# YanhaoWu/UMGen

Hardware: AMD Instinct MI355X
Metric: scene_tokens_per_sec (higher is better)
Workload: dtype bf16; 1 GPU; UMGen_large --infer_task video, 5-frame rollout, 1 scene(s)/GPU, T=20 history frames, top-k 5/5/16 sampling, rule_constrain; scenes_per_gpu=1, history_frames=20, input_history_frames=20

## Files before the change

umgen_amd/_lib.py:

```python
from __future__ import annotations

import ctypes as C
import os
import shutil
import subprocess

HERE = os.path.dirname(os.path.abspath(__file__))
CSRC = os.path.join(HERE, "csrc")
LIB_PATH = os.environ.get("UMGEN_LIB_PATH") or os.path.join(HERE, "libumgen_hip.so")
SOURCES = ["engine.hip", "gemm.hip", "gemm256.hip", "attn.hip", "gemv.hip", "oar_engine.hip", "oar_engine_wide.hip", "decode_batched.hip", "rowops.hip", "frame.hip", "tokenizers.hip", "vqdec.hip", "debug_api.hip"]
EXPORTS = ["umgen_create", "umgen_load_tensor", "umgen_finalize_weights", "umgen_rollout", "umgen_frame",
           "umgen_set_profiling", "umgen_get_timings", "umgen_last_error", "umgen_version", "umgen_destroy",
           "umgen_tokenize_ego", "umgen_detokenize_ego", "umgen_tokenize_boxes", "umgen_detokenize_boxes",
           "umgen_vq_create", "umgen_vq_load_tensor", "umgen_vq_finalize", "umgen_vq_decode", "umgen_vq_last_error", "umgen_vq_destroy",
           "umgen_dbg_linear", "umgen_dbg_attn_spatial", "umgen_dbg_attn_temporal", "umgen_dbg_attn_decode", "umgen_dbg_gemv", "umgen_dbg_gemm_bench", "umgen_dbg_oar_step", "umgen_dbg_sample_topk", "umgen_dbg_batched_layer_bench",
           "umgen_dbg_rows", "umgen_dbg_attn_decode_batched", "umgen_dbg_sample", "umgen_dbg_collision",
           "umgen_dbg_gemv_modes", "umgen_dbg_gemv_resid", "umgen_dbg_attn_partial", "umgen_dbg_decode_layer"]

HEADERS = ("common.h", "kernels.h", "frame.h", "oar_common.h", "bg_queue.h", "bg_worker.h", "gemm256_body.h", "attn_body.h", "rowops_body.h", "frame_body.h")

PREC_FP32, PREC_BF16, PREC_FP16 = 0, 1, 2
DT_F32, DT_BF16, DT_F16, DT_F64 = 0, 1, 2, 3


class Config(C.Structure):
    _fields_ = [(n, C.c_int32) for n in (
        "abi_version", "n_embd", "n_head", "n_ego_tar_layer", "n_ego_ca_layer", "n_map_tar_layer", "n_box_tar_layer",
        "n_tar_layer", "n_oar_layer", "pose_vocab", "map_vocab", "bbox3d_vocab", "img_vocab", "aux_vocab",
        "n_map_embd", "n_img_embd", "max_frame_len", "task_num", "task_id", "precision", "max_batch",
        "max_cond_frames", "device", "use_graphs")]


class VQConfig(C.Structure):
    _fields_ = [("n_embed", C.c_int32), ("embed_dim", C.c_int32), ("z_channels", C.c_int32), ("ch", C.c_int32), ("out_ch", C.c_int32),
                ("n_levels", C.c_int32), ("ch_mult", C.c_int32 * 8), ("num_res_blocks", C.c_int32), ("n_attn_res", C.c_int32),
                ("attn_resolutions", C.c_int32 * 4), ("resolution", C.c_int32), ("post_quant_ks", C.c_int32), ("post_quant_pad", C.c_int32),
                ("token_h", C.c_int32), ("token_w", C.c_int32), ("device", C.c_int32)]


class Sampling(C.Structure):
    _fields_ = [("method", C.c_int32), ("top_k", C.c_int32), ("top_k_map", C.c_int32), ("topk_image", C.c_int32),
                ("p", C.c_float), ("p_map", C.c_float), ("temperature", C.c_float),
                ("rule_constrain", C.c_int32), ("merge_ar_tar", C.c_int32), ("only_ar", C.c_int32),
                ("seeds", C.POINTER(C.c_uint64))]


class Trace(C.Structure):
    _fields_ = [("cond", C.POINTER(C.c_float)), ("ego_logits", C.POINTER(C.c_float)),
                ("logits_map", C.POINTER(C.c_float)), ("logits_bbox3d", C.POINTER(C.c_float)),
                ("logits_image", C.POINTER(C.c_float)),
                ("forced_pose", C.POINTER(C.c_int64)), ("forced_map", C.POINTER(C.c_int64)),
                ("forced_bbox3d", C.POINTER(C.c_int64)), ("forced_image", C.POINTER(C.c_int64)),
                ("counters", C.POINTER(C.c_int32)),
                ("given_map", C.POINTER(C.c_int64)), ("given_bbox3d", C.POINTER(C.c_int64))]


class Timings(C.Structure):
    _fields_ = [("total_ms", C.c_double), ("ego_ms", C.c_double), ("tar_ms", C.c_double), ("oar_ms", C.c_double),
                ("frames", C.c_int64), ("oar_steps", C.c_int64), ("oar_kernels", C.c_int64),
                ("gemm_ms", C.c_double), ("gemm_launches", C.c_int64), ("gemm_flops", C.c_double), ("oar_bytes", C.c_double),
                ("attn_ms", C.c_double), ("attn_launches", C.c_int64), ("attn_flops", C.c_double),
                ("bg_ms", C.c_double), ("overlapped_frames", C.c_int64),
                ("layers_ms", C.c_double), ("layers_launches", C.c_int64), ("decode_engine", C.c_int32), ("engine_fallback", C.c_int32),
                ("decode_batched", C.c_int32), ("decode_lanes", C.c_int32), ("prefix_passes", C.c_int64)]


def hipcc_path() -> str:
    p = shutil.which("hipcc") or "/opt/rocm/bin/hipcc"
    if not os.path.exists(p):
        raise RuntimeError("hipcc not found: cannot build libumgen_hip.so")
    return p


def source_hash() -> str:
    import hashlib
    h = hashlib.sha256()
    files = [os.path.join(CSRC, s) for s in SOURCES] + [os.path.join(CSRC, x) for x in HEADERS] + \
        [os.path.join(os.path.dirname(HERE), "include", "umgen.h")]
    for f in files:
        h.update(os.path.basename(f).encode())
        h.update(open(f, "rb").read())
    h.update(" ".join(HIPCC_FLAGS).encode())
    return h.hexdigest()[:16]


HIPCC_FLAGS = ["--offload-arch=gfx950", "-O3", "-std=c++17", "-fPIC", "-shared", "-Wno-unused-value", "-mllvm", "-amdgpu-mfma-vgpr-form=1"]


def build_library(force: bool = False, verbose: bool = False) -> str:
    srcs = [os.path.join(CSRC, s) for s in SOURCES]
    want = source_hash()
    stamp = LIB_PATH + ".srchash"
    if not force and os.path.exists(LIB_PATH) and os.path.exists(stamp) and open(stamp).read().strip() == want:
        return LIB_PATH
    import hashlib
    from concurrent.futures import ThreadPoolExecutor
    objdir = os.path.join(CSRC, ".obj")
    os.makedirs(objdir, exist_ok=True)
    hdr = b"".join(open(os.path.join(CSRC, x), "rb").read() for x in HEADERS) + \
        open(os.path.join(os.path.dirname(HERE), "include", "umgen.h"), "rb").read()
    cflags = [f for f in HIPCC_FLAGS if f != "-shared"]

# ... 141 lines not shown
```

umgen_amd/csrc/engine.hip:

```cpp
#include <hip/hip_runtime.h>

#include <algorithm>
#include <cmath>
#include <cstddef>
#include <cstdarg>
#include <cstdio>
#include <chrono>
#include <cstring>
#include <map>
#include <string>
#include <type_traits>
#include <vector>

#include "../../include/umgen.h"
#include "bg_queue.h"
#include "frame.h"
#include "kernels.h"

using namespace umgen;

namespace umgen { thread_local BgRecorder* g_bg_rec = nullptr; }

#define HIPCHK(e, call)                                                                              \
    do {                                                                                             \
// ... 31 lines not shown
    std::vector<TarW> stk[4];
    std::vector<SubW> oar;
    std::vector<DecW> dec;
    float *ln_ego_tar = nullptr, *ln_ego = nullptr, *ln_tar = nullptr, *ln_oar = nullptr, *ln_map_tar = nullptr, *ln_box_tar = nullptr;
    void *head_ego = nullptr, *head_ar_map = nullptr, *head_ar_box = nullptr, *head_tar_box = nullptr, *head_ar_img = nullptr;
    void *map_fc = nullptr, *map_proj = nullptr, *img_fc = nullptr, *img_proj = nullptr;
    float *map_cb = nullptr, *img_cb = nullptr;
    EmbedTables tb{};
    float *X = nullptr, *mapfeat = nullptr, *warped_last = nullptr, *cond = nullptr, *pose_diff = nullptr, *pego = nullptr;
    void *A = nullptr, *QKV = nullptr, *VT = nullptr, *Hb = nullptr;
    float *xdec = nullptr, *qdec = nullptr, *part = nullptr, *hdec = nullptr, *logits = nullptr, *logits_tar = nullptr, *qkv3 = nullptr;
    void* kvcache = nullptr;
    void* vtcache = nullptr;
    long vt_layer_stride = 0, vt_scene_stride = 0;
    long kv_layer_stride = 0, kv_scene_stride = 0;
    int Lmax = kAttnSplit * kAttnChunk, S_pad = 2240;
    int *d_pose = nullptr, *d_pose_shift = nullptr, *d_map = nullptr, *d_box = nullptr, *d_img = nullptr;
    int *d_tokens = nullptr, *d_prev_box = nullptr, *d_forced = nullptr, *d_counters = nullptr, *d_nboxes = nullptr, *d_ego_tok = nullptr;
    unsigned char* d_control = nullptr;
    double* d_boxes = nullptr;
    unsigned long long* d_seeds = nullptr;
    OarState* d_state = nullptr;
    bool overlap = false, overlap_suspended = false;
    bool conc_stacks = false;
    int last_B = 0;
    float last_full_pre_ms = 0.f, last_oar_ms = 0.f;
    int overlap_mode = 1;
    hipStream_t bg_stream = nullptr;
    struct Work { float* X; void *A, *QKV, *VT, *Hb; float* mapfeat; };
    Work w_main{}, w_side[2] = {};
    hipStream_t side_stream[2] = {nullptr, nullptr};
    hipEvent_t ev_side_in = nullptr, ev_side_done[2] = {nullptr, nullptr};
    void set_work(const Work& w) { X = w.X; A = w.A; QKV = w.QKV; VT = w.VT; Hb = w.Hb; mapfeat = w.mapfeat; }
    hipStream_t full_stream = nullptr;
    hipEvent_t ev_pre_done = nullptr;
    hipEvent_t ev_tar_done = nullptr, ev_bg_done = nullptr, ev_bg0 = nullptr;
    bool bg_pending = false;
    bool bg_engine = false;
    BgQueue* d_bgq = nullptr;
    struct BgHead { unsigned w[4]; EmbedTables tb; } bg_head{};
    BgRecorder bg_rec;
    std::vector<unsigned> bg_state_host;
    hipEvent_t ev_drain0 = nullptr, ev_drain1 = nullptr;
    std::vector<void*> tcache[4];
    bool grow_cache = true;
    int tcache_state = 0;
    struct Prefix {
        bool valid = false, has_ego = false;
        int B = 0, P = 0, Tfull = 0;
        std::vector<int> pose, map, box, img;
        std::vector<int> pose_next;
    } px;
    std::vector<int> px_up[4], px_pshift;
    std::vector<float> px_pdiff;
    hipEvent_t ev[4] = {nullptr, nullptr, nullptr, nullptr};
    umgen_timings tm{};
    bool profiling = false;
    int rows_per_block = -1;
    bool dbg_same_layer = false;
    hipGraphExec_t step_graph[4][kAttnSplit + 1] = {};
    int step_graph_B = 0;
    std::vector<std::pair<hipEvent_t, hipEvent_t>> gemm_ev, attn_ev, layer_ev;
    size_t gemm_ev_used = 0, attn_ev_used = 0, layer_ev_used = 0;
    struct EngStream { bool ok = false; int NG = 0; unsigned char map[16]; };
    bool eng_enabled = false, eng_fallback = false;
    EngStream eng_fg, eng_full;
    OarLayerDev* d_layers = nullptr;
    unsigned long long *eng_gx = nullptr, *eng_gloc = nullptr;
    unsigned int *eng_ticket = nullptr, *eng_err = nullptr;
    std::vector<void*> eng_wp2;
    std::vector<void*> eng_wf2;
    unsigned long long* eng_stamps = nullptr;
    size_t eng_gloc_bytes = 0;
    bool wide_enabled = false;
    OarLayerDev* d_layers_wide = nullptr;
    std::vector<void*> wide_wp2;
    unsigned long long* wide_gran = nullptr;
    unsigned int *wide_ticket = nullptr, *wide_err = nullptr;
    unsigned long long* wide_stamps = nullptr;
    bool use_wide(int B) const { return wide_enabled && tsz == 2 && B <= 4; }
    void* burn_buf = nullptr;
    int fg_xcds = 8;
    unsigned eng_epoch = 16u;
    int step_graph_NG = -1;
    bool in_capture = false;
    const EngStream* eng_for(hipStream_t s) const {
        if (!eng_enabled) return nullptr;
        const EngStream* es = (full_stream && s == full_stream) ? &eng_full : &eng_fg;
        return es->ok ? es : nullptr;
    }
    double gemm_flops_pending = 0, attn_flops_pending = 0;
    int batched_min = 24;
    float *xfrag = nullptr, *afrag = nullptr, *hfrag = nullptr;
    bool use_batched(int B) const {
        return tsz == 2 && (in_lanes || (batched_min > 0 && B >= batched_min)) && B <= kRowsMaxM && E % 32 == 0 && E <= 768;
    }
    static constexpr int kMaxLanes = 8;
    struct DecLane {
        hipStream_t s = nullptr;
        hipEvent_t done = nullptr;
        OarState* st = nullptr;
        float *xfrag = nullptr, *afrag = nullptr, *hfrag = nullptr;
        hipGraphExec_t graph[4][3] = {};
    };
    DecLane lane[kMaxLanes];
    hipEvent_t ev_lane_fork = nullptr;
    int lanes_env = -1;
    int lane_graph_B = 0, lane_graph_n = 0;
    bool in_lanes = false;
    int lane_count(int B) const {
        if (!use_batched(B) || !lane[0].s) return 1;
        int n = lanes_env > 0 ? lanes_env : std::min(4, std::max(B >= 24 ? 2 : 1, (B + 15) / 16));
        return std::max(1, std::min(std::min(n, kMaxLanes), B));
    }
    hipError_t launch_status = hipSuccess;

    int fail(int code, const char* fmt, ...) {
        char buf[512];
        va_list ap;
        va_start(ap, fmt);
        vsnprintf(buf, sizeof(buf), fmt, ap);
        va_end(ap);
        err = buf;
        return code;
    }
};

namespace {

int dev_alloc(umgen_engine* e, void** p, size_t bytes) {
    HIPCHK(e, hipMalloc(p, bytes ? bytes : 16));
    e->allocs.push_back(*p);
    return 0;
}
template <typename P>
int dalloc(umgen_engine* e, P** p, size_t n) { return dev_alloc(e, reinterpret_cast<void**>(p), n * sizeof(P)); }

void reg(umgen_engine* e, const std::string& key, void* dst, std::vector<int64_t> shape, int kind, bool optional = false) {
    e->slots[key] = Slot{dst, std::move(shape), kind, false, optional};
}

int alloc_f32(umgen_engine* e, const std::string& key, float** p, std::vector<int64_t> shape) {
    size_t n = 1;
    for (auto d : shape) n *= (size_t)d;
    if (int rc = dalloc(e, p, n)) return rc;
    reg(e, key, *p, shape, 0);
    return 0;
}
int alloc_w(umgen_engine* e, const std::string& key, void** p, std::vector<int64_t> shape) {
    size_t n = 1;
    for (auto d : shape) n *= (size_t)d;
    if (int rc = dev_alloc(e, p, n * e->tsz)) return rc;
    reg(e, key, *p, shape, 1);
    return 0;
}

int alloc_attn(umgen_engine* e, const std::string& pre, AttnW& a) {
    const int64_t E = e->E;
    if (int rc = alloc_w(e, pre + ".c_attn.weight", &a.Wqkv, {3 * E, E})) return rc;
    if (int rc = alloc_f32(e, pre + ".c_attn.bias", &a.bqkv, {3 * E})) return rc;
    if (int rc = alloc_w(e, pre + ".c_proj.weight", &a.Wo, {E, E})) return rc;
    return alloc_f32(e, pre + ".c_proj.bias", &a.bo, {E});
}
int alloc_mlp(umgen_engine* e, const std::string& pre, MlpW& m) {
    const int64_t E = e->E;
    if (int rc = alloc_w(e, pre + ".c_fc.weight", &m.Wfc, {4 * E, E})) return rc;
// ... 403 lines not shown
                }
                e->tcache_state = -1;
                return false;
            }
    }
    e->tcache_state = 1;
    return true;
}

struct FrameIO {
    int B, T;
    const int *pose, *map, *box, *img;
    const int* ctrl_pose;
    const unsigned char* control_slot;
    int frame_idx;
    const umgen_sampling* smp;
    const umgen_trace* trace;
    int* out_tokens;
    int cond_cap = 0;
    bool next_follows = false;
    bool next_has_ctrl_pose = false;
    const int* given_map = nullptr;
    const int* given_box = nullptr;
};

bool prefix_matches(const umgen_engine* e, const FrameIO& io) {
    const umgen_engine::Prefix& px = e->px;
    if (!px.valid || io.trace || io.B != px.B || io.T != px.Tfull || px.P != io.T - 1 || px.P < 1) return false;
    if (!io.ctrl_pose && !px.has_ego) return false;
    const int S[4] = {kNPose, kNMap, kNBox, kNImg};
    const int* cur[4] = {io.pose, io.map, io.box, io.img};
    const std::vector<int>* old[4] = {&px.pose, &px.map, &px.box, &px.img};
    for (int m = 0; m < 4; ++m)
        for (int b = 0; b < io.B; ++b)
            if (memcmp(cur[m] + (size_t)b * io.T * S[m], old[m]->data() + (size_t)b * px.P * S[m], (size_t)px.P * S[m] * sizeof(int))) return false;
    for (int b = 0; b < io.B; ++b)
        if (memcmp(io.pose + ((size_t)b * io.T + px.P) * kNPose, &px.pose_next[(size_t)b * 3], 3 * sizeof(int))) return false;
    return true;
}

void decode_pose_shift(const int* pose, const int* ego, int B, int Tn, std::vector<int>& pshift, std::vector<float>& pdiff) {
    pshift.resize((size_t)B * Tn * 3);
    pdiff.resize((size_t)B * Tn * 3);
    for (int b = 0; b < B; ++b)
        for (int t = 0; t < Tn; ++t)
            for (int a = 0; a < 3; ++a) {
                const int v = (t + 1 < Tn) ? pose[((size_t)b * Tn + t + 1) * 3 + a] : ego[b * 3 + a];
                pshift[((size_t)b * Tn + t) * 3 + a] = v;
                pdiff[((size_t)b * Tn + t) * 3 + a] = decode_pose_value(v, a);
            }
}

struct DecView {
    hipStream_t stream;
    float *xdec, *qdec, *logits, *logits_tar, *cond, *xfrag, *afrag, *hfrag;
    void* kvcache;
    int *d_tokens, *d_prev_box, *d_nboxes;
    unsigned char* d_control;
    double* d_boxes;
    unsigned long long* d_seeds;
    OarState* d_state;
};
DecView current_view(const umgen_engine* e) {
    return DecView{e->stream, e->xdec, e->qdec, e->logits, e->logits_tar, e->cond, e->xfrag, e->afrag, e->hfrag, e->kvcache,
                   e->d_tokens, e->d_prev_box, e->d_nboxes, e->d_control, e->d_boxes, e->d_seeds, e->d_state};
}
void apply_view(umgen_engine* e, const DecView& v) {
    e->stream = v.stream; e->xdec = v.xdec; e->qdec = v.qdec; e->logits = v.logits; e->logits_tar = v.logits_tar; e->cond = v.cond;
    e->xfrag = v.xfrag; e->afrag = v.afrag; e->hfrag = v.hfrag; e->kvcache = v.kvcache; e->d_tokens = v.d_tokens; e->d_prev_box = v.d_prev_box;
    e->d_nboxes = v.d_nboxes; e->d_control = v.d_control; e->d_boxes = v.d_boxes; e->d_seeds = v.d_seeds; e->d_state = v.d_state;
}
DecView lane_view(const umgen_engine* e, const DecView& all, const umgen_engine::DecLane& ln, int b0) {
    const long E = e->E;
    DecView v = all;
    v.stream = ln.s; v.d_state = ln.st; v.xfrag = ln.xfrag; v.afrag = ln.afrag; v.hfrag = ln.hfrag;
    v.xdec = all.xdec + b0 * E; v.qdec = all.qdec + b0 * E; v.logits = all.logits + (long)b0 * 8192;
    v.logits_tar = all.logits_tar + (long)b0 * kNBox * e->cfg.bbox3d_vocab; v.cond = all.cond + (long)b0 * kSeq * E;
    v.kvcache = static_cast<unsigned char*>(all.kvcache) + (size_t)b0 * e->kv_scene_stride * e->tsz;
    v.d_tokens = all.d_tokens + (long)b0 * kTokPerFrame; v.d_prev_box = all.d_prev_box + (long)b0 * kNBox; v.d_nboxes = all.d_nboxes + b0;
    v.d_control = all.d_control + (long)b0 * kSlots; v.d_boxes = all.d_boxes + (long)b0 * 64 * 10; v.d_seeds = all.d_seeds + b0;
    return v;
}

template <typename T>
int enqueue_step(umgen_engine* e, int B, int mod, int ns, const umgen_trace* tr, int j) {
    const int E = e->E;
    hipStream_t st = e->stream;
    const bool time_layers = e->profiling && !e->in_capture && !e->in_lanes;
    if (time_layers) {
        if (e->layer_ev_used == e->layer_ev.size()) {
            hipEvent_t a0, a1;
            hipEventCreate(&a0);
            hipEventCreate(&a1);
            e->layer_ev.emplace_back(a0, a1);
        }
        hipEventRecord(e->layer_ev[e->layer_ev_used].first, st);
    }
    if (int rc = oar_layers<T>(e, B, ns)) return rc;
    if (time_layers) hipEventRecord(e->layer_ev[e->layer_ev_used++].second, st);
    static FILE* dump = getenv("UMGEN_DEBUG_DUMP_X") ? fopen(getenv("UMGEN_DEBUG_DUMP_X"), "wb") : nullptr;
    if (dump && tr == nullptr && !e->cfg.use_graphs) {
        std::vector<float> hx((size_t)E);
        hipMemcpyAsync(hx.data(), e->xdec, (size_t)E * 4, hipMemcpyDeviceToHost, st);
        hipStreamSynchronize(st);
        fwrite(hx.data(), 4, E, dump);
        fflush(dump);
    }
    SampleArgs sa{};
    sa.st = e->d_state; sa.tb = e->tb; sa.logits = e->logits; sa.logits_tar = e->logits_tar; sa.ld_logits = 8192; sa.ld_tar = e->cfg.bbox3d_vocab;
    sa.cond = e->cond; sa.x_next = e->xdec; sa.tokens = e->d_tokens; sa.prev_box = e->d_prev_box; sa.control_slot = e->d_control;
    sa.boxes = e->d_boxes; sa.n_boxes = e->d_nboxes; sa.seeds = e->d_seeds; sa.forced = e->d_forced; sa.counters = e->d_counters;
    if (mod == 0) {
        launch_fixed_token(st, sa, B);
    } else {
        const void* head = mod == 1 ? e->head_ar_map : (mod == 2 ? e->head_ar_box : e->head_ar_img);
        const int V = mod == 1 ? e->cfg.map_vocab : (mod == 2 ? e->cfg.bbox3d_vocab : e->cfg.img_vocab);
        bool head_done = false;
        if constexpr (sizeof(T) == 2) {
            if (e->use_batched(B)) {
                RowsArgs r{};
                r.x = e->xfrag; r.M = B; r.ln_w = e->ln_oar; r.W = head; r.N = V; r.K = E; r.mode = ROWS_F32; r.out = e->logits; r.ldo = sa.ld_logits; r.E = E;
                launch_rows_mfma<T>(e->stream, r);
                head_done = true;
            }
        }
        if (!head_done) gemv<T>(e, e->xdec, E, e->ln_oar, head, nullptr, V, E, B, GEMV_OUT_F32, e->logits, sa.ld_logits);
        if (tr) {
            float* dst = mod == 1 ? tr->logits_map : (mod == 2 ? tr->logits_bbox3d : tr->logits_image);
            const int k = mod == 1 ? j - kMapC0 : (mod == 2 ? j - kBoxC0 : j - kImgC0);
            if (dst) HIPCHK(e, hipMemcpyAsync(dst + (size_t)k * V, e->logits, (size_t)V * 4, hipMemcpyDeviceToHost, st));
        }
        sa.mod = mod;
        sa.vocab = V;
        launch_sample_token(st, sa, B);
    }
    return 0;
}

template <typename T>
int launch_prefix(umgen_engine* e, const FrameIO& io, const std::vector<int>& ego) {
    const int B = io.B, Tn = io.T;
    const int Tnext = std::min(Tn + 1, io.cond_cap);
    const int off = (Tn + 1 > io.cond_cap) ? 1 : 0;
    const int P = Tnext - 1;
    if (P < 1 || Tnext > e->cfg.max_cond_frames) return 0;
    umgen_engine::Prefix& px = e->px;
    px.valid = false;
    px.B = B; px.P = P; px.Tfull = Tnext; px.has_ego = !io.next_has_ctrl_pose;
    const int S[4] = {kNPose, kNMap, kNBox, kNImg};
    const int* cur[4] = {io.pose, io.map, io.box, io.img};
    std::vector<int>* keep[4] = {&px.pose, &px.map, &px.box, &px.img};
    std::vector<int>* up[4] = {&e->px_up[0], &e->px_up[1], &e->px_up[2], &e->px_up[3]};
    for (int m = 0; m < 4; ++m) {
        keep[m]->assign((size_t)B * P * S[m], 0);
        up[m]->assign((size_t)B * Tnext * S[m], 0);
        for (int b = 0; b < B; ++b) {
            const int* src = cur[m] + ((size_t)b * Tn + off) * S[m];
            memcpy(keep[m]->data() + (size_t)b * P * S[m], src, (size_t)P * S[m] * sizeof(int));
            memcpy(up[m]->data() + (size_t)b * Tnext * S[m], src, (size_t)P * S[m] * sizeof(int));
        }
    }
    px.pose_next.assign(ego.begin(), ego.end());
    for (int b = 0; b < B; ++b)
        for (int a = 0; a < 3; ++a) (*up[0])[((size_t)b * Tnext + P) * 3 + a] = ego[b * 3 + a];
    std::vector<int> zero((size_t)B * 3, 0);
    decode_pose_shift(up[0]->data(), zero.data(), B, Tnext, e->px_pshift, e->px_pdiff);

    hipStream_t fg = e->stream, bg = e->bg_engine ? e->stream : e->bg_stream;
    if (!e->bg_engine) {
        HIPCHK(e, hipEventRecord(e->ev_tar_done, fg));
        HIPCHK(e, hipStreamWaitEvent(bg, e->ev_tar_done, 0));
    }
    HIPCHK(e, hipMemcpyAsync(e->d_pose, up[0]->data(), up[0]->size() * 4, hipMemcpyHostToDevice, bg));
    HIPCHK(e, hipMemcpyAsync(e->d_map, up[1]->data(), up[1]->size() * 4, hipMemcpyHostToDevice, bg));
    HIPCHK(e, hipMemcpyAsync(e->d_box, up[2]->data(), up[2]->size() * 4, hipMemcpyHostToDevice, bg));
    HIPCHK(e, hipMemcpyAsync(e->d_img, up[3]->data(), up[3]->size() * 4, hipMemcpyHostToDevice, bg));
    HIPCHK(e, hipMemcpyAsync(e->d_pose_shift, e->px_pshift.data(), e->px_pshift.size() * 4, hipMemcpyHostToDevice, bg));
    HIPCHK(e, hipMemcpyAsync(e->pose_diff, e->px_pdiff.data(), e->px_pdiff.size() * 4, hipMemcpyHostToDevice, bg));
    const WindowTokens ws{e->d_pose_shift, e->d_map, e->d_box, e->d_img, B, P, Tnext, 0};
    if (e->bg_engine) {
        BgRecorder rec;
        g_bg_rec = &rec;
        if (px.has_ego) run_stack<T>(e, STACK_EGO, WindowTokens{e->d_pose, e->d_map, e->d_box, e->d_img, B, P, Tnext, 0}, 1);
        run_stack<T>(e, STACK_MAP, ws, 1);
        run_stack<T>(e, STACK_BOX, ws, 1);
        run_stack<T>(e, STACK_TAR, ws, 1);
        g_bg_rec = nullptr;
        if (rec.failed || rec.ops.empty() || rec.ops.size() > (size_t)kBgMaxOps) {
            if (getenv("UMGEN_DEBUG_TIMING")) fprintf(stderr, "[umgen] background pass not recordable (%s): this frame's successor computes its whole window\n", rec.failed ? rec.failed : "op count");
            return 0;
        }
        bool same = rec.ops.size() == e->bg_rec.ops.size();
        for (size_t i = 0; same && i < rec.ops.size(); ++i) same = memcmp(&rec.ops[i].h, &e->bg_rec.ops[i].h, sizeof(BgOpHead)) == 0;
        e->bg_rec = std::move(rec);
        e->bg_head.w[0] = (unsigned)e->bg_rec.ops.size(); e->bg_head.w[1] = 0u; e->bg_head.w[2] = (unsigned)(getenv("UMGEN_BG_MARGIN_US") ? atoi(getenv("UMGEN_BG_MARGIN_US")) * 100 : 1000); e->bg_head.w[3] = 0u;
        e->bg_head.tb = e->tb;
        static_assert(offsetof(BgQueue, tb) == 16 && offsetof(BgQueue, state) == 16 + sizeof(EmbedTables), "BgQueue header layout");
        HIPCHK(e, hipMemcpyAsync(&e->d_bgq->n_ops, &e->bg_head, sizeof(e->bg_head), hipMemcpyHostToDevice, fg));
        HIPCHK(e, hipMemsetAsync(&e->d_bgq->state[0][0], 0, sizeof(e->d_bgq->state) + sizeof(e->d_bgq->arrive), fg));
        if (!same) HIPCHK(e, hipMemcpyAsync(&e->d_bgq->est[0], e->bg_rec.est.data(), e->bg_rec.est.size() * sizeof(unsigned), hipMemcpyHostToDevice, fg));
        HIPCHK(e, hipMemcpyAsync(&e->d_bgq->ops[0], e->bg_rec.ops.data(), e->bg_rec.ops.size() * sizeof(BgOp), hipMemcpyHostToDevice, fg));
        e->bg_pending = true;
        return 0;
    }
    HIPCHK(e, hipEventRecord(e->ev_bg0, bg));
    e->stream = bg;
    if (px.has_ego) run_stack<T>(e, STACK_EGO, WindowTokens{e->d_pose, e->d_map, e->d_box, e->d_img, B, P, Tnext, 0}, 1);
    run_stack<T>(e, STACK_MAP, ws, 1);
    run_stack<T>(e, STACK_BOX, ws, 1);
    run_stack<T>(e, STACK_TAR, ws, 1);
    e->stream = fg;
    HIPCHK(e, hipEventRecord(e->ev_bg_done, bg));
    e->bg_pending = true;
    px.valid = true;
    return 0;
}

// ... 18 lines not shown
        const auto tw0 = std::chrono::steady_clock::now();
        HIPCHK(e, hipEventSynchronize(e->ev_bg_done));
        const double waited = std::chrono::duration<double, std::milli>(std::chrono::steady_clock::now() - tw0).count();
        if (waited > 25.0 && e->overlap_mode != 2) e->overlap_suspended = true;
        if (getenv("UMGEN_DEBUG_TIMING")) fprintf(stderr, "[umgen] waited %.1f ms for the background pass\n", waited);
        float bms = 0.f;
        hipEventElapsedTime(&bms, e->ev_bg0, e->ev_bg_done);
        e->tm.bg_ms += bms;
        e->bg_pending = false;
    }
    const bool use_px = prefix_matches(e, io);
    if (e->last_B != B) { e->last_B = B; e->last_full_pre_ms = 0.f; }
    const bool hides = e->overlap_mode == 2 || e->last_full_pre_ms <= 0.f || (e->bg_engine ? 2.3f * e->last_full_pre_ms < e->last_oar_ms : 3.3f * e->last_full_pre_ms < 0.95f * e->last_oar_ms);
    const bool ov_active = e->overlap && !e->overlap_suspended && hides && !e->profiling && !tr && (B == 1 || e->overlap_mode == 2);
    hipStream_t const pre = e->full_stream ? e->full_stream : fg;
    hipStream_t const dec = (e->full_stream && !ov_active) ? e->full_stream : fg;
    st = pre;
    e->stream = pre;
    HIPCHK(e, hipMemcpyAsync(e->d_pose, io.pose, (size_t)B * Tn * 3 * 4, hipMemcpyHostToDevice, st));
    HIPCHK(e, hipMemcpyAsync(e->d_map, io.map, (size_t)B * Tn * kNMap * 4, hipMemcpyHostToDevice, st));
    HIPCHK(e, hipMemcpyAsync(e->d_box, io.box, (size_t)B * Tn * kNBox * 4, hipMemcpyHostToDevice, st));
    HIPCHK(e, hipMemcpyAsync(e->d_img, io.img, (size_t)B * Tn * kNImg * 4, hipMemcpyHostToDevice, st));
    std::vector<unsigned long long> seeds(B);
    for (int b = 0; b < B; ++b) seeds[b] = io.smp->seeds ? io.smp->seeds[b] : 0ull;
    HIPCHK(e, hipMemcpyAsync(e->d_seeds, seeds.data(), (size_t)B * 8, hipMemcpyHostToDevice, st));
    std::vector<int> forced_host;
    if (forced) {
        forced_host.resize(kTokPerFrame);
        for (int i = 0; i < kNPose; ++i) forced_host[i] = (int)tr->forced_pose[i];
        for (int i = 0; i < kNMap; ++i) forced_host[kOffMap + i] = (int)tr->forced_map[i];
        for (int i = 0; i < kNBox; ++i) forced_host[kOffBox + i] = (int)tr->forced_bbox3d[i];
        for (int i = 0; i < kNImg; ++i) forced_host[kOffImg + i] = (int)tr->forced_image[i];
        HIPCHK(e, hipMemcpyAsync(e->d_forced, forced_host.data(), (size_t)kTokPerFrame * 4, hipMemcpyHostToDevice, st));
    }
    HIPCHK(e, hipMemsetAsync(e->d_counters, 0, 8 * sizeof(int), st));
    HIPCHK(e, hipMemsetAsync(e->d_nboxes, 0, (size_t)B * sizeof(int), st));

    const bool fg_write = !e->overlap && e->grow_cache && io.next_follows && io.cond_cap > 0 && Tn + 1 <= io.cond_cap &&
                          Tn + 1 <= e->cfg.max_cond_frames && !tr && ensure_tcache(e);
    const int t0 = use_px ? Tn - 1 : 0, Tc = use_px ? 1 : Tn, cmode = use_px ? (fg_write ? 4 : 2) : (fg_write ? 3 : 0);
    e->px.valid = false;
    WindowTokens w{e->d_pose, e->d_map, e->d_box, e->d_img, B, Tc, Tn, t0};
    std::vector<int> ego(B * 3);
    HIPCHK(e, hipEventRecord(e->ev[0], st));
    if (io.ctrl_pose) {
        for (int i = 0; i < B * 3; ++i) ego[i] = io.ctrl_pose[i];
    } else {
        run_ego<T>(e, w, sp, io.frame_idx, forced, tr ? tr->ego_logits : nullptr, cmode);
        HIPCHK(e, hipMemcpyAsync(ego.data(), e->d_ego_tok, (size_t)B * 3 * 4, hipMemcpyDeviceToHost, st));
        HIPCHK(e, hipStreamSynchronize(st));
    }
    HIPCHK(e, hipEventRecord(e->ev[1], st));
    std::vector<int> pshift;
    std::vector<float> pdiff;
    decode_pose_shift(io.pose, ego.data(), B, Tn, pshift, pdiff);
    HIPCHK(e, hipMemcpyAsync(e->d_pose_shift, pshift.data(), pshift.size() * 4, hipMemcpyHostToDevice, st));
    HIPCHK(e, hipMemcpyAsync(e->pose_diff, pdiff.data(), pdiff.size() * 4, hipMemcpyHostToDevice, st));
    std::vector<int> tok0((size_t)B * kTokPerFrame, 0);
    std::vector<int> prevbox((size_t)B * kNBox);
    for (int b = 0; b < B; ++b) {
        for (int a = 0; a < 3; ++a) tok0[(size_t)b * kTokPerFrame + a] = ego[b * 3 + a];
        memcpy(&prevbox[(size_t)b * kNBox], io.box + ((size_t)b * Tn + (Tn - 1)) * kNBox, kNBox * sizeof(int));
        if (io.given_map) memcpy(&tok0[(size_t)b * kTokPerFrame + kOffMap], io.given_map + (size_t)b * kNMap, kNMap * sizeof(int));
        if (io.given_box) memcpy(&tok0[(size_t)b * kTokPerFrame + kOffBox], io.given_box + (size_t)b * kNBox, kNBox * sizeof(int));
    }
    const int given_end = io.given_box ? kBoxEos + 1 : (io.given_map ? kMapEos + 1 : kPoseEos + 1);
    HIPCHK(e, hipMemcpyAsync(e->d_tokens, tok0.data(), tok0.size() * 4, hipMemcpyHostToDevice, st));
    HIPCHK(e, hipMemcpyAsync(e->d_prev_box, prevbox.data(), prevbox.size() * 4, hipMemcpyHostToDevice, st));
    if (io.control_slot) HIPCHK(e, hipMemcpyAsync(e->d_control, io.control_slot, (size_t)B * kSlots, hipMemcpyHostToDevice, st));
    int j_begin = 0, j_end = kImgEos;
    if (const char* dbg = getenv("UMGEN_DEBUG_OAR_STEPS")) {
        int a0 = 0, b0 = kImgEos;
        if (sscanf(dbg, "%d:%d", &a0, &b0) == 2 && a0 >= 0 && b0 <= kImgEos && a0 < b0) { j_begin = a0; j_end = b0; }
    }
    if (e->wide_enabled && e->eng_epoch > 0xE0000000u) {
        HIPCHK(e, hipDeviceSynchronize());
        HIPCHK(e, hipMemset(e->wide_gran, 0, oar_engine_wide_granules() * 8));
        e->eng_epoch = 16u;
    }
    if (e->eng_enabled && e->eng_epoch > 0xE0000000u) {
        HIPCHK(e, hipDeviceSynchronize());
        HIPCHK(e, hipMemset(e->eng_gx, 0, (size_t)e->cfg.max_batch * kEngE * 8));
        HIPCHK(e, hipMemset(e->eng_gloc, 0, e->eng_gloc_bytes));
        e->eng_epoch = 16u;
    }
    OarState s0{j_begin, io.frame_idx, forced ? 1 : 0, io.control_slot ? 1 : 0, 0, e->eng_epoch, sp};
    e->eng_epoch += (unsigned)(kImgEos + 1) * kEpochPerStep;
    HIPCHK(e, hipMemcpyAsync(e->d_state, &s0, sizeof(s0), hipMemcpyHostToDevice, st));
    const int n_lanes = (sizeof(T) == 2 && !tr) ? e->lane_count(B) : 1;
    for (int l = 0; l < n_lanes && n_lanes > 1; ++l) HIPCHK(e, hipMemcpyAsync(e->lane[l].st, &s0, sizeof(s0), hipMemcpyHostToDevice, st));

    WindowTokens ws{e->d_pose_shift, e->d_map, e->d_box, e->d_img, B, Tc, Tn, t0};
    if ((use_px || (e->conc_stacks && !e->profiling)) && e->side_stream[0]) {
        struct Restore { umgen_engine* e; hipStream_t s; ~Restore() { e->stream = s; e->set_work(e->w_main); } } restore{e, st};
        HIPCHK(e, hipEventRecord(e->ev_side_in, st));
        const int side_stack[2] = {STACK_MAP, STACK_BOX};
        for (int i = 0; i < 2; ++i) {
            HIPCHK(e, hipStreamWaitEvent(e->side_stream[i], e->ev_side_in, 0));
            e->stream = e->side_stream[i];
            e->set_work(e->w_side[i]);
            run_stack<T>(e, side_stack[i], ws, cmode);
            launch_cond_rows(e->stream, side_stack[i], B, Tc, E, e->X, i == 0 ? e->ln_map_tar : e->ln_box_tar, i == 0 ? e->warped_last : nullptr,
                             e->cond);
            HIPCHK(e, hipEventRecord(e->ev_side_done[i], e->side_stream[i]));
        }
        e->stream = st;
        e->set_work(e->w_main);
        run_stack<T>(e, STACK_TAR, ws, cmode);
        launch_cond_rows(st, STACK_TAR, B, Tc, E, e->X, e->ln_tar, nullptr, e->cond);
        for (int i = 0; i < 2; ++i) HIPCHK(e, hipStreamWaitEvent(st, e->ev_side_done[i], 0));
    } else {
        run_stack<T>(e, STACK_MAP, ws, cmode);
        launch_cond_rows(st, STACK_MAP, B, Tc, E, e->X, e->ln_map_tar, e->warped_last, e->cond);
        run_stack<T>(e, STACK_BOX, ws, cmode);
        launch_cond_rows(st, STACK_BOX, B, Tc, E, e->X, e->ln_box_tar, nullptr, e->cond);
        run_stack<T>(e, STACK_TAR, ws, cmode);
        launch_cond_rows(st, STACK_TAR, B, Tc, E, e->X, e->ln_tar, nullptr, e->cond);
    }
    if (tr && tr->cond) HIPCHK(e, hipMemcpyAsync(tr->cond, e->cond, (size_t)kSeq * E * 4, hipMemcpyDeviceToHost, st));
    HIPCHK(e, hipEventRecord(e->ev[2], st));
    if (fg_write) {
        umgen_engine::Prefix& px = e->px;
        px.B = B; px.P = Tn; px.Tfull = Tn + 1; px.has_ego = !io.ctrl_pose;
        px.pose.assign(io.pose, io.pose + (size_t)B * Tn * kNPose);
        px.map.assign(io.map, io.map + (size_t)B * Tn * kNMap);
        px.box.assign(io.box, io.box + (size_t)B * Tn * kNBox);
        px.img.assign(io.img, io.img + (size_t)B * Tn * kNImg);
        px.pose_next.assign(ego.begin(), ego.end());
        px.valid = true;
    }

    if (dec != pre) {
        HIPCHK(e, hipEventRecord(e->ev_pre_done, pre));
        HIPCHK(e, hipStreamWaitEvent(dec, e->ev_pre_done, 0));
    }
    st = dec;
    e->stream = dec;
    launch_first_input(st, B, E, e->tb.tske + (long)e->cfg.task_id * E, e->cond, e->xdec);
    {
        GemmArgs g{};
        g.P = e->head_tar_box; g.Q = e->cond + (long)kBoxC0 * E; g.Mi = e->cfg.bbox3d_vocab; g.Nj = kNBox; g.K = E; g.ldp = E; g.ldq = E;
        g.strideP = 0; g.strideQ = (long)kSeq * E; g.batch = B; g.mode = GEMM_STORE_F32; g.out = e->logits_tar; g.ldo = e->cfg.bbox3d_vocab;
        g.strideO = (long)kNBox * e->cfg.bbox3d_vocab;
        launch_gemm_valu<T, float>(st, g);
    }
    if (ov_active && io.next_follows) {
        const auto tp0 = std::chrono::steady_clock::now();
        if (int rc = launch_prefix<T>(e, io, ego)) return rc;
        if (getenv("UMGEN_DEBUG_TIMING"))
            fprintf(stderr, "[umgen] host time to enqueue the background pass: %.1f ms\n",
                    std::chrono::duration<double, std::milli>(std::chrono::steady_clock::now() - tp0).count());
    }
    const char* ppe = getenv("UMGEN_PREFIX_PASS");
    const bool prefix_pass_off = ppe && ppe[0] == '0';
    OarState s1 = s0;
    if (given_end > kPoseEos + 1 && !prefix_pass_off && (!e->overlap || e->bg_engine) && j_begin == 0) {
        if (int rc = run_prefix_prefill<T>(e, B, given_end)) return rc;
        j_begin = given_end - 1;
        s1.step = j_begin;
        HIPCHK(e, hipMemcpyAsync(e->d_state, &s1, sizeof(s1), hipMemcpyHostToDevice, st));
        for (int l = 0; l < n_lanes && n_lanes > 1; ++l) HIPCHK(e, hipMemcpyAsync(e->lane[l].st, &s1, sizeof(s1), hipMemcpyHostToDevice, st));
        e->tm.prefix_passes += 1;
    }
    const int steps_run = j_end - j_begin;
    const bool graphs = e->cfg.use_graphs && !tr && !e->profiling;
    const bool batched = sizeof(T) == 2 && e->use_batched(B);
// ... 36 lines not shown
        for (int j = j_begin; j < j_end; ++j) {
            const int mod = kind_of(j);
            int same = 1;
            while (same < 16 && j + same < j_end && kind_of(j + same) == mod) ++same;
            const int run = !lane_graphs ? 1 : (same >= 16 ? 16 : (same >= 4 ? 4 : 1));
            const int ri = run == 16 ? 2 : (run == 4 ? 1 : 0);
            for (int l = 0; l < n_lanes; ++l) {
                umgen_engine::DecLane& ln = e->lane[l];
                apply_view(e, lane_view(e, all, ln, b0s[l]));
                const bool timed = e->profiling && l == 0;
                if (timed) {
                    if (e->layer_ev_used == e->layer_ev.size()) {
                        hipEvent_t a0, a1;
                        hipEventCreate(&a0);
                        hipEventCreate(&a1);
                        e->layer_ev.emplace_back(a0, a1);
                    }
                    hipEventRecord(e->layer_ev[e->layer_ev_used].first, ln.s);
                }
                if (lane_graphs) {
                    hipGraphExec_t& ge = ln.graph[mod][ri];
                    if (!ge) {
                        hipGraph_t g;
                        HIPCHK(e, hipStreamBeginCapture(ln.s, hipStreamCaptureModeThreadLocal));
                        e->in_capture = true;
                        int crc = 0;
                        for (int r = 0; r < run && !crc; ++r) crc = enqueue_step<T>(e, nbs[l], mod, 1, nullptr, 0);
                        e->in_capture = false;
                        if (crc) return crc;
                        HIPCHK(e, hipStreamEndCapture(ln.s, &g));
                        HIPCHK(e, hipGraphInstantiate(&ge, g, nullptr, nullptr, 0));
                        HIPCHK(e, hipGraphDestroy(g));
                    }
                    HIPCHK(e, hipGraphLaunch(ge, ln.s));
                } else if (int rc = enqueue_step<T>(e, nbs[l], mod, 1, nullptr, j)) {
                    return rc;
                }
                if (timed) {
                    hipEventRecord(e->layer_ev[e->layer_ev_used++].second, ln.s);
                    e->tm.layers_launches += run - 1;
                }
                e->tm.oar_kernels += (int64_t)run * (5 * (int64_t)e->oar.size() + (mod == 0 ? 1 : (mod == 2 ? 3 : 2)));
            }
            j += run - 1;
        }
        for (int l = 0; l < n_lanes; ++l) {
            HIPCHK(e, hipEventRecord(e->lane[l].done, e->lane[l].s));
            HIPCHK(e, hipStreamWaitEvent(st, e->lane[l].done, 0));
        }
        j_begin = j_end;
    }
    for (int j = j_begin; j < j_end; ++j) {
        auto kind_of = [given_end](int jj) {
            if (jj < given_end) return 0;
            return (jj >= kMapC0 && jj < kMapEos) ? 1 : (jj >= kBoxC0 && jj < kBoxEos) ? 2 : (jj >= kImgC0 && jj < kImgEos) ? 3 : 0;
        };
        const int mod = kind_of(j);
        const int ns = attn_nsplit(j + 1);
        const int gkey = (eng || batched) ? 0 : ns;
        if (graphs) {
            int run = 1;
            if (eng || batched) {
                int same = 1;
                while (same < 16 && j + same < j_end) {
                    if (kind_of(j + same) != mod) break;
                    ++same;
                }
                run = same >= 16 ? 16 : (same >= 4 ? 4 : 1);
            }
            hipGraphExec_t& ge = e->step_graph[mod][(eng || batched) ? (run == 16 ? 2 : (run == 4 ? 1 : 0)) : gkey];
            if (!ge) {
                hipGraph_t g;
                HIPCHK(e, hipStreamBeginCapture(st, hipStreamCaptureModeThreadLocal));
                e->in_capture = true;
                int crc = 0;
                for (int r = 0; r < run && !crc; ++r) crc = enqueue_step<T>(e, B, mod, ns, nullptr, 0);
                e->in_capture = false;
                if (crc) return crc;
                HIPCHK(e, hipStreamEndCapture(st, &g));
                HIPCHK(e, hipGraphInstantiate(&ge, g, nullptr, nullptr, 0));
                HIPCHK(e, hipGraphDestroy(g));
            }
            HIPCHK(e, hipGraphLaunch(ge, st));
            e->tm.oar_kernels += (int64_t)(run - 1) * ((eng ? (wide ? B : 1) : 5 * (int64_t)e->oar.size()) + (mod == 0 ? 1 : (mod == 2 ? 3 : 2)));
            j += run - 1;
        } else if (int rc = enqueue_step<T>(e, B, mod, ns, tr, j)) {
            return rc;
        }
        e->tm.oar_kernels += (eng ? (wide ? B : 1) : 5 * (int64_t)e->oar.size()) + (mod == 0 ? 1 : (mod == 2 ? 3 : 2));
    }
    e->tm.oar_steps += steps_run;
    const bool drained = e->bg_engine && e->bg_pending;
    if (drained) {
        HIPCHK(e, hipEventRecord(e->ev_drain0, st));
        OarEngineArgs a{};
        a.NG = 8; a.R = 2; a.D = 4; a.B = 1; a.bg = e->d_bgq; a.bg_only = 1;
        a.st = e->d_state; a.ticket = e->eng_ticket; a.err = e->eng_err;
        memcpy(a.xcc_group, e->eng_fg.map, 16);
        a.fp16 = std::is_same<T, f16_t>::value ? 1 : 0;
        HIPCHK(e, launch_oar_engine(st, a));
        HIPCHK(e, hipEventRecord(e->ev_drain1, st));
        e->bg_state_host.assign((size_t)kBgMaxWorkers * 4, 0u);
        HIPCHK(e, hipMemcpyAsync(e->bg_state_host.data(), &e->d_bgq->state[0][0], sizeof(e->d_bgq->state), hipMemcpyDeviceToHost, st));
    }
    HIPCHK(e, hipEventRecord(e->ev[3], st));
    HIPCHK(e, hipMemcpyAsync(io.out_tokens, e->d_tokens, (size_t)B * kTokPerFrame * 4, hipMemcpyDeviceToHost, st));
    int counters[8] = {};
    HIPCHK(e, hipMemcpyAsync(counters, e->d_counters, 8 * sizeof(int), hipMemcpyDeviceToHost, st));
    unsigned eng_err = 0;
    if (eng) HIPCHK(e, hipMemcpyAsync(&eng_err, wide ? e->wide_err : e->eng_err, sizeof(unsigned), hipMemcpyDeviceToHost, st));
    HIPCHK(e, hipStreamSynchronize(st));
    {
        const hipError_t le = e->launch_status != hipSuccess ? e->launch_status : hipGetLastError();
        e->launch_status = hipSuccess;
        if (le != hipSuccess) return e->fail(UMGEN_E_HIP, "a kernel launch of this frame was refused: %s", hipGetErrorString(le));
    }
    if (drained) {
        e->bg_pending = false;
        float dms = 0.f;
        hipEventElapsedTime(&dms, e->ev_drain0, e->ev_drain1);
        e->tm.bg_ms += dms;
        for (int wk = 0; wk < kBgMaxWorkers; ++wk)
            if (e->bg_state_host[(size_t)wk * 4] < e->bg_rec.ops.size()) {
                e->px.valid = false;
                if (getenv("UMGEN_DEBUG_TIMING")) {
                    fprintf(stderr, "[umgen] worker states (op, units done | arrived):");
                    for (int k = 0; k < kBgMaxWorkers; ++k) fprintf(stderr, " %u:%x", e->bg_state_host[(size_t)k * 4], e->bg_state_host[(size_t)k * 4 + 1]);
                    const unsigned o0 = e->bg_state_host[(size_t)wk * 4];
                    unsigned arr[4] = {};
                    (void)hipMemcpy(arr, &e->d_bgq->arrive[o0 > 0 ? o0 - 1 : 0], sizeof(arr), hipMemcpyDeviceToHost);
                    const BgOpHead& h = e->bg_rec.ops[o0].h;
                    fprintf(stderr, "\n[umgen] arrivals from op %u on: %u %u %u %u; op %u: kind %d mode %d units %d chunk %d i0..3 %d %d %d %d\n", o0 > 0 ? o0 - 1 : 0, arr[0], arr[1], arr[2], arr[3], o0,
                            h.kind, h.mode, h.n_units, h.chunk, h.i0, h.i1, h.i2, h.i3);
                }
                return e->fail(UMGEN_E_HIP, "background pass incomplete: worker %d stopped at op %u of %zu", wk, e->bg_state_host[(size_t)wk * 4], e->bg_rec.ops.size());
            }
        e->px.valid = true;
        if (getenv("UMGEN_DEBUG_TIMING")) {
            fprintf(stderr, "[umgen] background pass: %zu ops, drain launch %.2f ms\n", e->bg_rec.ops.size(), dms);
            std::vector<unsigned> est(e->bg_rec.ops.size());
            if (hipMemcpy(est.data(), &e->d_bgq->est[0], est.size() * 4, hipMemcpyDeviceToHost) == hipSuccess) {
                double by_kind[8] = {}, gemm_by_mode[4] = {};
                for (size_t i = 0; i < est.size(); ++i) {
                    const BgOpHead& h = e->bg_rec.ops[i].h;
                    const double us = std::ceil((double)h.n_units / 128.0) * ((double)est[i] - 20.0) / 1.125 / 100.0;
                    by_kind[h.kind & 7] += us;
                    if (h.kind == BG_GEMM) gemm_by_mode[h.mode & 3] += us;
                }
                fprintf(stderr, "[umgen] per-worker time by kind (ms, upper bound): gemm %.1f (store %.1f, resid %.1f, vt %.1f) ln %.1f attn_s %.1f attn_t %.1f embed %.1f warp %.1f\n", by_kind[BG_GEMM] / 1e3,
                        gemm_by_mode[GEMM_STORE] / 1e3, gemm_by_mode[GEMM_RESID] / 1e3, gemm_by_mode[GEMM_VT] / 1e3, by_kind[BG_LN] / 1e3, by_kind[BG_ATTN_S] / 1e3, by_kind[BG_ATTN_T] / 1e3,
                        by_kind[BG_EMBED] / 1e3, by_kind[BG_WARP] / 1e3);
            }
        }
    }
    if (eng_err) {
        (void)hipMemset(wide ? e->wide_err : e->eng_err, 0, sizeof(unsigned));
        return e->fail(UMGEN_E_HIP, "decode engine gave up waiting for hand-off tag 0x%08x (is another persistent kernel using this GPU?)", eng_err);
    }
    if (tr && tr->counters) memcpy(tr->counters, counters, sizeof(counters));
    float ms;
    hipEventElapsedTime(&ms, e->ev[0], e->ev[1]); e->tm.ego_ms += ms;
    hipEventElapsedTime(&ms, e->ev[1], e->ev[2]); e->tm.tar_ms += ms;
    hipEventElapsedTime(&ms, e->ev[2], e->ev[3]); e->tm.oar_ms += ms;
    e->last_oar_ms = ms;
    if (!use_px) {
        float pre = 0.f;
        hipEventElapsedTime(&pre, e->ev[0], e->ev[2]);
        e->last_full_pre_ms = pre;
    }
    hipEventElapsedTime(&ms, e->ev[0], e->ev[3]); e->tm.total_ms += ms;
    e->tm.frames += 1;
    e->tm.decode_engine = eng ? (wide ? 3 : 1) : 0;
// ... 199 lines not shown
    HIPCHK(e, gemm256_prepare());
    const char* de_env = getenv("UMGEN_DECODE_ENGINE");
    const char* ov_env = getenv("UMGEN_OVERLAP");
    const bool engine_wanted = cfg->precision != UMGEN_PREC_FP32 && cfg->n_embd == kEngE && cfg->n_head == kEngH && cfg->n_oar_layer <= 64 &&
                               cfg->max_batch <= 256 && !(de_env && de_env[0] == '0') && !(ov_env && ov_env[0] != '0');
    if (engine_wanted) {
        HIPCHK(e, hipStreamCreate(&e->stream));
        HIPCHK(e, oar_engine_prepare());
        unsigned* d_cnt = nullptr;
        HIPCHK(e, hipMalloc(&d_cnt, 64));
        umgen_engine::EngStream& es = e->eng_fg;
        es.ok = true;
        for (int rep = 0; rep < 2 && es.ok; ++rep) {
            unsigned cnt[16] = {};
            if (hipMemsetAsync(d_cnt, 0, 64, e->stream) != hipSuccess || launch_oar_engine_census(e->stream, 8, d_cnt) != hipSuccess ||
                hipMemcpyAsync(cnt, d_cnt, 64, hipMemcpyDeviceToHost, e->stream) != hipSuccess || hipStreamSynchronize(e->stream) != hipSuccess) {
                (void)hipGetLastError();
                es.ok = false;
                break;
            }
            if (getenv("UMGEN_DEBUG_TIMING")) {
                fprintf(stderr, "[umgen] engine census:");
                for (int x = 0; x < 16; ++x) fprintf(stderr, " %u", cnt[x]);
                fprintf(stderr, "\n");
            }
            int groups = 0;
            unsigned char map[16];
            for (int x = 0; x < 16; ++x) {
                map[x] = 0xff;
                if (cnt[x] == (unsigned)kEngGroup) map[x] = (unsigned char)groups++;
                else if (cnt[x] != 0) es.ok = false;
            }
            if (groups != 8 || (rep == 1 && memcmp(map, es.map, 16))) es.ok = false;
            memcpy(es.map, map, 16);
        }
        (void)hipFree(d_cnt);
        es.NG = 8;
        e->eng_enabled = es.ok;
        if (!es.ok) {
            e->eng_fallback = true;
            fprintf(stderr, "[umgen] WARNING: the XCD-resident decode engine cannot be used on device %d (its census did not find 32 workgroups on each "
                            "of 8 XCDs); decode steps run as five launches per layer (~30 %% slower at one scene per GPU)\n", cfg->device);
            HIPCHK(e, hipStreamDestroy(e->stream));
            e->stream = nullptr;
        }
    }
    const char* dw_env = getenv("UMGEN_DECODE_WIDE");
    if (cfg->precision != UMGEN_PREC_FP32 && cfg->n_embd == kWideE && cfg->n_head == kWideE / kHeadDim && cfg->n_oar_layer <= 64 &&
        cfg->max_batch <= std::max(0, std::min(4, dw_env ? atoi(dw_env) : 1)) && !(ov_env && ov_env[0] != '0')) {
        HIPCHK(e, hipStreamCreate(&e->stream));
        HIPCHK(e, oar_engine_wide_prepare());
        unsigned* d_cnt = nullptr;
        HIPCHK(e, hipMalloc(&d_cnt, 64));
        bool ok = true;
        for (int rep2 = 0; rep2 < 2 && ok; ++rep2) {
            unsigned cnt[16] = {};
            if (hipMemsetAsync(d_cnt, 0, 64, e->stream) != hipSuccess || launch_oar_engine_wide_census(e->stream, d_cnt) != hipSuccess ||
                hipMemcpyAsync(cnt, d_cnt, 64, hipMemcpyDeviceToHost, e->stream) != hipSuccess || hipStreamSynchronize(e->stream) != hipSuccess) {
                (void)hipGetLastError();
                ok = false;
                break;
            }
            int groups = 0;
            for (int x = 0; x < 16; ++x) {
                if (cnt[x] == (unsigned)kEngGroup) ++groups;
                else if (cnt[x] != 0) ok = false;
            }
            if (groups != 8) ok = false;
        }
        (void)hipFree(d_cnt);
        e->wide_enabled = ok;
        if (!ok) {
            fprintf(stderr, "[umgen] WARNING: the chip-wide decode engine cannot be used on device %d (its census did not find one workgroup on each of 256 "
                            "CUs); decode steps run as five launches per layer\n", cfg->device);
            HIPCHK(e, hipStreamDestroy(e->stream));
            e->stream = nullptr;
        }
    }
    e->overlap = cfg->max_cond_frames >= 2 && !e->eng_enabled && !e->wide_enabled;
    if (ov_env) { e->overlap_mode = ov_env[0] - '0'; e->overlap = cfg->max_cond_frames >= 2 && ov_env[0] != '0'; }
    const char* be_env = getenv("UMGEN_BG_ENGINE");
    e->bg_engine = e->eng_enabled && cfg->max_batch == 1 && cfg->max_cond_frames >= 2 && cfg->max_cond_frames <= 32 && !ov_env && !(be_env && be_env[0] == '0');
    if (e->bg_engine) { e->overlap = true; e->overlap_mode = 1; }
    int bg_cus = 64;
    if (const char* bc = getenv("UMGEN_BG_CUS")) bg_cus = std::max(32, std::min(128, atoi(bc)));
    if (e->bg_engine) {
        void* qp = nullptr;
        if (int rc = dev_alloc(e, &qp, sizeof(BgQueue))) return rc;
        e->d_bgq = reinterpret_cast<BgQueue*>(qp);
        HIPCHK(e, hipMemset(e->d_bgq, 0, sizeof(BgQueue)));
        HIPCHK(e, hipEventCreate(&e->ev_drain0));
        HIPCHK(e, hipEventCreate(&e->ev_drain1));
    }
    if (e->overlap && !e->bg_engine) {
        hipDeviceProp_t prop;
        HIPCHK(e, hipGetDeviceProperties(&prop, cfg->device));
        const int ncu = prop.multiProcessorCount;
        if (ncu < 2 * bg_cus) e->overlap = false;
        else {
            std::vector<uint32_t> mbg((ncu + 31) / 32, 0u), mfg((ncu + 31) / 32, 0u);
            int fg_cus = ncu - bg_cus;
            if (const char* fc = getenv("UMGEN_FG_CUS")) fg_cus = std::max(32, std::min(ncu - bg_cus, atoi(fc)));
            e->fg_xcds = fg_cus / 32;
            for (int cu = 0; cu < ncu; ++cu) {
                if (cu < bg_cus) mbg[cu / 32] |= 1u << (cu % 32);
                else if (cu < bg_cus + fg_cus) mfg[cu / 32] |= 1u << (cu % 32);
            }
            if (hipExtStreamCreateWithCUMask(&e->stream, (uint32_t)mfg.size(), mfg.data()) != hipSuccess ||
                hipExtStreamCreateWithCUMask(&e->bg_stream, (uint32_t)mbg.size(), mbg.data()) != hipSuccess) {
                (void)hipGetLastError();
                if (e->stream) { hipStreamDestroy(e->stream); e->stream = nullptr; }
                if (e->bg_stream) { hipStreamDestroy(e->bg_stream); e->bg_stream = nullptr; }
                e->overlap = false;
            } else {
                HIPCHK(e, hipStreamCreateWithFlags(&e->full_stream, hipStreamNonBlocking));
                HIPCHK(e, hipEventCreate(&e->ev_pre_done));
                HIPCHK(e, hipEventCreate(&e->ev_tar_done));
                HIPCHK(e, hipEventCreate(&e->ev_bg_done));
                HIPCHK(e, hipEventCreate(&e->ev_bg0));
            }
        }
    }
    if (!e->stream) HIPCHK(e, hipStreamCreate(&e->stream));
    for (auto& ev : e->ev) HIPCHK(e, hipEventCreate(&ev));
    e->E = cfg->n_embd;
    e->H = cfg->n_head;
    if (const char* sl = getenv("UMGEN_DEBUG_SAME_LAYER")) e->dbg_same_layer = sl[0] == '1';
    if (const char* rb = getenv("UMGEN_ROWS_PER_BLOCK")) e->rows_per_block = rb[0] - '0';
    e->tsz = cfg->precision == UMGEN_PREC_FP32 ? 4 : 2;
    const int64_t E = e->E;
    const std::string t = "transformer.";
    float* tmp;
    if (int rc = alloc_f32(e, t + "egoe.weight", &tmp, {3, E})) return rc; e->tb.egoe = tmp;
    if (int rc = alloc_f32(e, t + "axe.weight", &tmp, {cfg->aux_vocab, E})) return rc; e->tb.axe = tmp;
    if (int rc = alloc_f32(e, t + "be.weight", &tmp, {cfg->bbox3d_vocab, E})) return rc; e->tb.be = tmp;
    if (int rc = alloc_f32(e, t + "tpe.weight", &tmp, {cfg->max_frame_len, E})) return rc; e->tb.tpe = tmp;
    if (int rc = alloc_f32(e, t + "spe.weight", &tmp, {kSeq, E})) return rc; e->tb.spe = tmp;
    if (int rc = alloc_f32(e, t + "tske.weight", &tmp, {cfg->task_num, E})) return rc; e->tb.tske = tmp;
    e->tb.E = e->E;
    const char* stack_name[4] = {"ego_tar", "map_tar", "box_tar", "TAR"};
    const int stack_n[4] = {cfg->n_ego_tar_layer, cfg->n_map_tar_layer, cfg->n_box_tar_layer, cfg->n_tar_layer};
    for (int s = 0; s < 4; ++s) {
        e->stk[s].resize(stack_n[s]);
        for (int i = 0; i < stack_n[s]; ++i) {
            const std::string pre = t + stack_name[s] + "." + std::to_string(i);
            TarW& b = e->stk[s][i];
            if (int rc = alloc_sub(e, pre, "ln_1", "spatial_attn_1", "ln_2", "mlp1", b.sub[0])) return rc;
            if (int rc = alloc_sub(e, pre, "ln_3", "temporal_attn", "ln_4", "mlp2", b.sub[1])) return rc;
            if (int rc = alloc_sub(e, pre, "ln_5", "spatial_attn_2", "ln_6", "mlp3", b.sub[2])) return rc;
        }
    }
    e->oar.resize(cfg->n_oar_layer);
    for (int i = 0; i < cfg->n_oar_layer; ++i)
        if (int rc = alloc_sub(e, t + "OAR." + std::to_string(i), "ln_1", "temporal_attn", "ln_2", "mlp", e->oar[i])) return rc;
    e->dec.resize(cfg->n_ego_ca_layer);
    for (int i = 0; i < cfg->n_ego_ca_layer; ++i) {
        const std::string pre = t + "ego_cross_attn." + std::to_string(i);
        DecW& d = e->dec[i];
        if (int rc = alloc_f32(e, pre + ".ln_1.weight", &d.ln1, {E})) return rc;
        if (int rc = alloc_attn(e, pre + ".self_attn", d.self)) return rc;
        if (int rc = alloc_f32(e, pre + ".ln_2.weight", &d.ln2, {E})) return rc;
        if (int rc = alloc_f32(e, pre + ".ln_3.weight", &d.ln3, {E})) return rc;
        if (int rc = alloc_w(e, pre + ".cross_attn.q_attn.weight", &d.Wq, {E, E})) return rc;
        if (int rc = alloc_f32(e, pre + ".cross_attn.q_attn.bias", &d.bq, {E})) return rc;
        if (int rc = dev_alloc(e, &d.Wkv, (size_t)2 * E * E * e->tsz)) return rc;
        if (int rc = dalloc(e, &d.bkv, (size_t)2 * E)) return rc;
// ... 74 lines not shown
            if (int rc = dalloc(e, &w.mapfeat, Bm * slots * kNMap * E)) return rc;
            HIPCHK(e, hipStreamCreateWithFlags(&e->side_stream[i], hipStreamNonBlocking));
            HIPCHK(e, hipEventCreate(&e->ev_side_done[i]));
        }
        HIPCHK(e, hipEventCreate(&e->ev_side_in));
    }
    if (int rc = dalloc(e, &e->warped_last, Bm * kNMap * E)) return rc;
    if (int rc = dalloc(e, &e->cond, Bm * kSeq * E)) return rc;
    if (int rc = dalloc(e, &e->pego, Bm * kSeq * E)) return rc;
    if (int rc = dalloc(e, &e->pose_diff, Bm * Tm * 3)) return rc;
    if (int rc = dalloc(e, &e->xdec, 3 * Bm * E)) return rc;
    if (int rc = dalloc(e, &e->qdec, 3 * Bm * E)) return rc;
    if (int rc = dalloc(e, &e->qkv3, 3 * Bm * 3 * E)) return rc;
    if (int rc = dalloc(e, &e->part, 3 * Bm * e->H * kAttnRec)) return rc;
    HIPCHK(e, hipMemset(e->part, 0, 3 * Bm * e->H * kAttnRec * sizeof(float)));
    if (int rc = dalloc(e, &e->hdec, 3 * Bm * 4 * E)) return rc;
    if (int rc = dalloc(e, &e->xfrag, (size_t)kRowsMaxM * E)) return rc;
    if (int rc = dalloc(e, &e->afrag, (size_t)kRowsMaxM * E)) return rc;
    if (int rc = dalloc(e, &e->hfrag, (size_t)kRowsMaxM * 4 * E)) return rc;
    HIPCHK(e, hipMemset(e->xfrag, 0, (size_t)kRowsMaxM * E * 4));
    HIPCHK(e, hipMemset(e->afrag, 0, (size_t)kRowsMaxM * E * 4));
    HIPCHK(e, hipMemset(e->hfrag, 0, (size_t)kRowsMaxM * 4 * E * 4));
    if (const char* bd = getenv("UMGEN_DECODE_BATCHED")) e->batched_min = atoi(bd);
    if (const char* dl = getenv("UMGEN_DECODE_LANES")) e->lanes_env = atoi(dl);
    if (e->tsz == 2 && Bm >= 2 && e->lanes_env != 1) {
        for (auto& ln : e->lane) {
            HIPCHK(e, hipStreamCreateWithFlags(&ln.s, hipStreamNonBlocking));
            HIPCHK(e, hipEventCreateWithFlags(&ln.done, hipEventDisableTiming));
            if (int rc = dalloc(e, &ln.st, (size_t)1)) return rc;
            if (int rc = dalloc(e, &ln.xfrag, (size_t)kRowsMaxM * E)) return rc;
            if (int rc = dalloc(e, &ln.afrag, (size_t)kRowsMaxM * E)) return rc;
            if (int rc = dalloc(e, &ln.hfrag, (size_t)kRowsMaxM * 4 * E)) return rc;
            HIPCHK(e, hipMemset(ln.xfrag, 0, (size_t)kRowsMaxM * E * 4));
            HIPCHK(e, hipMemset(ln.afrag, 0, (size_t)kRowsMaxM * E * 4));
            HIPCHK(e, hipMemset(ln.hfrag, 0, (size_t)kRowsMaxM * 4 * E * 4));
        }
        HIPCHK(e, hipEventCreateWithFlags(&e->ev_lane_fork, hipEventDisableTiming));
    }
    if (int rc = dalloc(e, &e->logits, 3 * Bm * 8192)) return rc;
    if (int rc = dalloc(e, &e->logits_tar, Bm * kNBox * (size_t)cfg->bbox3d_vocab)) return rc;
    e->kv_scene_stride = (long)e->Lmax * 2 * E;
    e->kv_layer_stride = (long)Bm * e->kv_scene_stride;
    if (int rc = dev_alloc(e, &e->kvcache, (size_t)cfg->n_oar_layer * e->kv_layer_stride * e->tsz)) return rc;
    HIPCHK(e, hipMemset(e->kvcache, 0, (size_t)cfg->n_oar_layer * e->kv_layer_stride * e->tsz));
    if ((UMGEN_ENG_MFMA & 16) && e->tsz == 2) {
        HIPCHK(e, hipMemset(e->kvcache, 0, (size_t)cfg->n_oar_layer * e->kv_layer_stride * e->tsz));
        e->vt_scene_stride = (long)e->H * kHeadDim * e->Lmax;
        e->vt_layer_stride = (long)Bm * e->vt_scene_stride;
        if (int rc = dev_alloc(e, &e->vtcache, (size_t)cfg->n_oar_layer * e->vt_layer_stride * e->tsz)) return rc;
        HIPCHK(e, hipMemset(e->vtcache, 0, (size_t)cfg->n_oar_layer * e->vt_layer_stride * e->tsz));
    }
    if (e->overlap && !ensure_tcache(e)) e->overlap = false;
    if (const char* gc = getenv("UMGEN_GROW_CACHE")) e->grow_cache = gc[0] != '0';
    if (int rc = dalloc(e, &e->d_pose, Bm * Tm * 3)) return rc;
    if (int rc = dalloc(e, &e->d_pose_shift, Bm * Tm * 3)) return rc;
    if (int rc = dalloc(e, &e->d_map, Bm * Tm * kNMap)) return rc;
    if (int rc = dalloc(e, &e->d_box, Bm * Tm * kNBox)) return rc;
    if (int rc = dalloc(e, &e->d_img, Bm * Tm * kNImg)) return rc;
    if (int rc = dalloc(e, &e->d_tokens, Bm * kTokPerFrame)) return rc;
    if (int rc = dalloc(e, &e->d_prev_box, Bm * kNBox)) return rc;
    if (int rc = dalloc(e, &e->d_forced, Bm * kTokPerFrame)) return rc;
    if (int rc = dalloc(e, &e->d_counters, (size_t)8)) return rc;
    if (int rc = dalloc(e, &e->d_nboxes, Bm)) return rc;
    if (int rc = dalloc(e, &e->d_ego_tok, Bm * 3)) return rc;
    if (int rc = dalloc(e, &e->d_control, Bm * kSlots)) return rc;
    if (int rc = dalloc(e, &e->d_boxes, Bm * 64 * 10)) return rc;
    if (int rc = dalloc(e, &e->d_seeds, Bm)) return rc;
    if (int rc = dalloc(e, &e->d_state, (size_t)1)) return rc;
    if (e->eng_enabled) {
        if (int rc = dalloc(e, &e->d_layers, (size_t)cfg->n_oar_layer)) return rc;
        std::vector<OarLayerDev> hl(cfg->n_oar_layer);
        for (int i = 0; i < cfg->n_oar_layer; ++i) {
            const SubW& w = e->oar[i];
            hl[i] = OarLayerDev{reinterpret_cast<const bf16_t*>(w.attn.Wqkv), reinterpret_cast<const bf16_t*>(w.attn.Wo),
                                reinterpret_cast<const bf16_t*>(w.mlp.Wfc), reinterpret_cast<const bf16_t*>(w.mlp.Wproj), nullptr,
                                w.attn.bqkv, w.attn.bo, w.ln_a, w.ln_b};
        }
        HIPCHK(e, hipMemcpy(e->d_layers, hl.data(), hl.size() * sizeof(OarLayerDev), hipMemcpyHostToDevice));
        e->eng_gloc_bytes = (size_t)16 * kEngLocStride * 8;
        if (int rc = dalloc(e, &e->eng_gx, Bm * kEngE)) return rc;
        if (int rc = dev_alloc(e, reinterpret_cast<void**>(&e->eng_gloc), e->eng_gloc_bytes)) return rc;
        if (int rc = dalloc(e, &e->eng_ticket, (size_t)16)) return rc;
        if (int rc = dalloc(e, &e->eng_err, (size_t)4)) return rc;
        HIPCHK(e, hipMemset(e->eng_ticket, 0, 64));
        if (getenv("UMGEN_DEBUG_TIMING") && !e->bg_engine) {
            if (int rc = dalloc(e, &e->eng_stamps, (size_t)16)) return rc;
            HIPCHK(e, hipMemset(e->eng_stamps, 0, 128));
        }
        HIPCHK(e, hipMemset(e->eng_gx, 0, Bm * kEngE * 8));
        HIPCHK(e, hipMemset(e->eng_gloc, 0, e->eng_gloc_bytes));
        HIPCHK(e, hipMemset(e->eng_err, 0, 16));
        if (const char* bs = getenv("UMGEN_DEBUG_BURN")) {
            int us = 0, mf = 0, sl = 0, kb = 0;
            if (sscanf(bs, "%d,%d,%d,%d", &us, &mf, &sl, &kb) == 4 && kb > 0) {
                if (int rc = dev_alloc(e, &e->burn_buf, (size_t)kb << 10)) return rc;
                HIPCHK(e, hipMemset(e->burn_buf, 1, (size_t)kb << 10));
            }
        }
        if (getenv("UMGEN_DEBUG_TIMING")) fprintf(stderr, "[umgen] decode engine: on (8 XCD groups)\n");
    }
    if (e->wide_enabled) {
        if (int rc = dalloc(e, &e->d_layers_wide, (size_t)cfg->n_oar_layer)) return rc;
        if (int rc = dalloc(e, &e->wide_gran, oar_engine_wide_granules())) return rc;
        if (int rc = dalloc(e, &e->wide_ticket, (size_t)16)) return rc;
        if (int rc = dalloc(e, &e->wide_err, (size_t)4)) return rc;
        HIPCHK(e, hipMemset(e->wide_gran, 0, oar_engine_wide_granules() * 8));
        HIPCHK(e, hipMemset(e->wide_ticket, 0, 64));
        HIPCHK(e, hipMemset(e->wide_err, 0, 16));
        if (getenv("UMGEN_DEBUG_TIMING")) {
            if (int rc = dalloc(e, &e->wide_stamps, (size_t)16)) return rc;
            HIPCHK(e, hipMemset(e->wide_stamps, 0, 128));
        }
    }
    return UMGEN_OK;
}

int umgen_load_tensor(umgen_engine* e, const char* key, const void* data, int32_t dtype, const int64_t* shape, int32_t ndim) {
    if (!e || !key || !data) return UMGEN_E_INVALID;
    auto it = e->slots.find(key);
    if (it == e->slots.end()) return 1;
    Slot& s = it->second;
    if ((size_t)ndim != s.shape.size()) return e->fail(UMGEN_E_INVALID, "%s: ndim %d, expected %zu", key, ndim, s.shape.size());
    size_t n = 1;
    for (int i = 0; i < ndim; ++i) {
        if (shape[i] != s.shape[i]) return e->fail(UMGEN_E_INVALID, "%s: dim %d is %lld, expected %lld", key, i, (long long)shape[i], (long long)s.shape[i]);
        n *= (size_t)shape[i];
    }
    if (dtype < 0 || dtype > UMGEN_DT_F64) return e->fail(UMGEN_E_INVALID, "%s: dtype %d", key, dtype);
    const bool to_bf16 = (s.kind == 2) || (s.kind == 1 && e->cfg.precision == UMGEN_PREC_BF16);
    if (s.kind == 1 && e->cfg.precision == UMGEN_PREC_FP16) {
        std::vector<f16_t> h(n);
        if (dtype == UMGEN_DT_F16) memcpy(h.data(), data, n * 2);
        else {
            unsigned overflow = 0;
            for (size_t i = 0; i < n; ++i) {
                const float v = load_as_f32(data, dtype, i);
                const uint16_t hb = f32_to_f16_bits_host(v);
                overflow |= (unsigned)(((hb & 0x7fffu) == 0x7c00u) & (std::fabs(v) <= 3.4e38f));
                memcpy(&h[i], &hb, 2);
            }
            if (overflow) {
                for (size_t i = 0; i < n; ++i) {
                    const float v = load_as_f32(data, dtype, i);
                    if (std::isfinite(v) && (f32_to_f16_bits_host(v) & 0x7fffu) == 0x7c00u)
                        return e->fail(UMGEN_E_INVALID, "%s[%zu] = %g does not fit fp16 (precision fp16 needs |w| < 65520)", key, i, (double)v);
                }
            }
        }
        HIPCHK(e, hipMemcpy(s.dst, h.data(), n * 2, hipMemcpyHostToDevice));
    } else if (to_bf16) {
        std::vector<bf16_t> h(n);
        if (dtype == UMGEN_DT_BF16) memcpy(h.data(), data, n * 2);
        else for (size_t i = 0; i < n; ++i) h[i] = f32_to_bf16(load_as_f32(data, dtype, i));
        HIPCHK(e, hipMemcpy(s.dst, h.data(), n * 2, hipMemcpyHostToDevice));
    } else {
        if (dtype == UMGEN_DT_F32) {
            HIPCHK(e, hipMemcpy(s.dst, data, n * 4, hipMemcpyHostToDevice));
        } else {
            std::vector<float> h(n);
            for (size_t i = 0; i < n; ++i) h[i] = load_as_f32(data, dtype, i);
            HIPCHK(e, hipMemcpy(s.dst, h.data(), n * 4, hipMemcpyHostToDevice));
        }
    }
    s.loaded = true;
    e->finalized = false;
    return UMGEN_OK;
// ... 186 lines not shown
    std::vector<int> frame_out((size_t)B * kTokPerFrame);
    for (int idx = 0; idx < new_frames; ++idx) {
        if (T_cur > cond_frames) {
            for (int m = 0; m < 4; ++m) {
                std::vector<int> nw((size_t)B * cond_frames * S[m]);
                for (int b = 0; b < B; ++b)
                    memcpy(&nw[(size_t)b * cond_frames * S[m]], &hist[m][((size_t)b * T_cur + (T_cur - cond_frames)) * S[m]],
                           (size_t)cond_frames * S[m] * sizeof(int));
                hist[m].swap(nw);
            }
            T_cur = cond_frames;
        }
        if (have_ctl && idx >= T_ctl) { have_ctl = false; have_box = false; have_given = false; control_test = 0; }
        if (have_box && idx >= T_ctl) have_box = false;
        if (have_given && idx >= T_ctl) have_given = false;
        std::vector<int> gm, gb;
        if (have_given) {
            gm.resize((size_t)B * kNMap);
            for (int b = 0; b < B; ++b)
                for (int i = 0; i < kNMap; ++i) gm[(size_t)b * kNMap + i] = (int)given_map[((size_t)b * T_ctl + idx) * kNMap + i];
            if (given_bbox3d) {
                gb.resize((size_t)B * kNBox);
                for (int b = 0; b < B; ++b)
                    for (int i = 0; i < kNBox; ++i) gb[(size_t)b * kNBox + i] = (int)given_bbox3d[((size_t)b * T_ctl + idx) * kNBox + i];
            }
        }
        std::vector<int> cp;
        std::vector<unsigned char> cs;
        if (have_ctl) {
            cp.resize((size_t)B * 3);
            for (int b = 0; b < B; ++b)
                for (int a = 0; a < 3; ++a) cp[b * 3 + a] = (int)ctrl_pose[((size_t)b * T_ctl + idx) * 3 + a];
        }
        if (have_box) {
            if (control_test) {
                cs.assign((size_t)B * kSlots, 0);
                for (int b = 0; b < B; ++b)
                    for (int i = 0; i < kNBox; ++i) {
                        const int64_t v = ctrl_bbox3d[((size_t)b * T_ctl + idx) * kNBox + i];
                        if (v != -1) { hist[2][((size_t)b * T_cur + (T_cur - 1)) * kNBox + i] = (int)v; cs[(size_t)b * kSlots + i / kSlotLen] = 1; }
                    }
            } else {
                return e->fail(UMGEN_E_UNSUPPORTED, "init_tokens['bbox3d'] without control_test is not a supported reference path");
            }
        }
        FrameIO io{B, T_cur, hist[0].data(), hist[1].data(), hist[2].data(), hist[3].data(), have_ctl ? cp.data() : nullptr,
                   cs.empty() ? nullptr : cs.data(), idx, sampling, nullptr, frame_out.data()};
        io.cond_cap = cond_frames;
        io.next_follows = idx + 1 < new_frames;
        io.next_has_ctrl_pose = have_ctl && idx + 1 < T_ctl;
        io.given_map = gm.empty() ? nullptr : gm.data();
        io.given_box = gb.empty() ? nullptr : gb.data();
        if (int rc = run_frame_any(e, io)) return rc;
        const int off[4] = {0, kOffMap, kOffBox, kOffImg};
        for (int m = 0; m < 4; ++m) {
            std::vector<int> nw((size_t)B * (T_cur + 1) * S[m]);
            for (int b = 0; b < B; ++b) {
                memcpy(&nw[(size_t)b * (T_cur + 1) * S[m]], &hist[m][(size_t)b * T_cur * S[m]], (size_t)T_cur * S[m] * sizeof(int));
                for (int i = 0; i < S[m]; ++i) {
                    const int v = frame_out[(size_t)b * kTokPerFrame + off[m] + i];
                    nw[((size_t)b * (T_cur + 1) + T_cur) * S[m] + i] = v;
                    out[m][((size_t)b * T_out + T_in + idx) * S[m] + i] = v;
                }
            }
            hist[m].swap(nw);
        }
        T_cur += 1;
    }
    return UMGEN_OK;
}

int umgen_dbg_oar_step(umgen_engine* e, int32_t B, int32_t L, const float* x_in, float* x_out, int32_t use_engine, int32_t unmasked) {
    if (!e || !x_in || !x_out) return UMGEN_E_INVALID;
    if (!e->finalized) return e->fail(UMGEN_E_STATE, "umgen_finalize_weights has not been called");
    if (e->cfg.precision == UMGEN_PREC_FP32) return e->fail(UMGEN_E_UNSUPPORTED, "16-bit engines only");
    if (B < 1 || B > e->cfg.max_batch || L < 0 || L >= e->Lmax) return e->fail(UMGEN_E_INVALID, "B=%d L=%d", B, L);
    if (use_engine != 0 && use_engine != 1 && use_engine != 3) return e->fail(UMGEN_E_INVALID, "use_engine %d (0: five launches per layer, 1: XCD-resident engine, 3: chip-wide engine)", use_engine);
    if (use_engine == 1 && !e->eng_enabled) return e->fail(UMGEN_E_UNSUPPORTED, "decode engine not available on this engine");
    if (e->eng_epoch > 0xE0000000u) {
        HIPCHK(e, hipDeviceSynchronize());
        if (e->eng_enabled) {
            HIPCHK(e, hipMemset(e->eng_gx, 0, (size_t)e->cfg.max_batch * kEngE * 8));
            HIPCHK(e, hipMemset(e->eng_gloc, 0, e->eng_gloc_bytes));
        }
        if (e->wide_enabled) HIPCHK(e, hipMemset(e->wide_gran, 0, oar_engine_wide_granules() * 8));
        e->eng_epoch = 16u;
    }
    const unsigned epoch = e->eng_epoch;
    e->eng_epoch += kEpochPerStep;
    hipStream_t const keep = e->stream;
    hipStream_t const st = (unmasked && e->full_stream) ? e->full_stream : e->stream;
    OarState s0{L, 0, 0, 0, 0, epoch, SamplerParams{}};
    HIPCHK(e, hipMemcpyAsync(e->d_state, &s0, sizeof(s0), hipMemcpyHostToDevice, st));
    HIPCHK(e, hipMemcpyAsync(e->xdec, x_in, (size_t)B * e->E * 4, hipMemcpyHostToDevice, st));
    const bool en = e->eng_enabled, wide_keep = e->wide_enabled;
    if (use_engine == 3 && !e->wide_enabled) return e->fail(UMGEN_E_UNSUPPORTED, "chip-wide decode engine not available on this engine");
    e->wide_enabled = wide_keep && use_engine == 3;
    e->eng_enabled = en && use_engine == 1;
    e->stream = st;
    const int lrc = e->cfg.precision == UMGEN_PREC_FP16 ? oar_layers<f16_t>(e, B, attn_nsplit(L + 1)) : oar_layers<bf16_t>(e, B, attn_nsplit(L + 1));
    e->stream = keep;
    e->eng_enabled = en;
    e->wide_enabled = wide_keep;
    if (lrc) return lrc;
    HIPCHK(e, hipMemcpyAsync(x_out, e->xdec, (size_t)B * e->E * 4, hipMemcpyDeviceToHost, st));
    unsigned eng_err = 0;
    if (use_engine) HIPCHK(e, hipMemcpyAsync(&eng_err, use_engine == 3 ? e->wide_err : e->eng_err, sizeof(unsigned), hipMemcpyDeviceToHost, st));
    HIPCHK(e, hipStreamSynchronize(st));
    if (eng_err) {
        (void)hipMemset(use_engine == 3 ? e->wide_err : e->eng_err, 0, sizeof(unsigned));
        return e->fail(UMGEN_E_HIP, "decode engine gave up waiting for hand-off tag 0x%08x", eng_err);
    }
    return UMGEN_OK;
}

int umgen_destroy(umgen_engine* e) {
    if (!e) return UMGEN_OK;
    (void)hipSetDevice(e->cfg.device);
    (void)hipDeviceSynchronize();
    if (e->wide_stamps) {
        unsigned long long st[16];
        if (hipMemcpy(st, e->wide_stamps, 128, hipMemcpyDeviceToHost) == hipSuccess && st[15]) {
            const char* nm[14] = {"wait x", "LN + qkv rows", "wait qkv", "attention", "wait waves", "quarter out + wait quarters", "merge + wait att", "c_proj", "wait x'",
                                  "LN + c_fc + GELU", "wait waves", "mlp partial sums", "wait partial sums", "add partials"};
            fprintf(stderr, "[umgen] chip-wide decode engine, rank 0 wave 0, us per layer over %llu layers:", st[15]);
            double tot = 0;
            for (int p = 0; p < 14; ++p) { fprintf(stderr, " %s %.2f", nm[p], (double)st[p] / 100.0 / (double)st[15]); tot += (double)st[p] / 100.0 / (double)st[15]; }
            fprintf(stderr, " | total %.2f\n", tot);
        }
    }
    if (e->eng_stamps) {
        unsigned long long st[16];
        if (hipMemcpy(st, e->eng_stamps, 128, hipMemcpyDeviceToHost) == hipSuccess && st[10]) {
            const char* nm[10] = {"wait x", "qkv rows", "wait qkv", "attention", "wait partials", "c_proj", "wait x'", "c_fc + partial sums", "wait partial sums", "add partials"};
            fprintf(stderr, "[umgen] decode engine, group 0 rank 0, us per item over %llu items:", st[10]);
            double tot = 0;
            for (int p = 0; p < 10; ++p) { fprintf(stderr, " %s %.2f", nm[p], (double)st[p] / 100.0 / (double)st[10]); tot += (double)st[p] / 100.0 / (double)st[10]; }
            fprintf(stderr, " (c_fc part %.2f)", (double)st[11] / 100.0 / (double)st[10]);
            fprintf(stderr, " | total %.2f\n", tot);
            if (st[15])
                fprintf(stderr, "[umgen] decode engine, prologue of a launch (%llu launches): kernel entry -> rank, step, epoch known %.2f us; kernel entry -> first item's q|k|v + parked mlp rows there %.2f us"
                        "; kernel entry -> first item's x, LN weights and q|k|v rows there %.2f us\n", st[15], (double)st[12] / 100.0 / (double)st[15],
                        (double)st[13] / 100.0 / (double)st[15], (double)st[14] / 100.0 / (double)st[15]);
        }
    }
    for (auto& row : e->step_graph)
        for (auto& g : row)
            if (g) hipGraphExecDestroy(g);
    for (auto& ln : e->lane) {
        for (auto& row : ln.graph)
            for (auto& g : row)
                if (g) hipGraphExecDestroy(g);
        if (ln.s) { hipStreamSynchronize(ln.s); hipStreamDestroy(ln.s); }
        if (ln.done) hipEventDestroy(ln.done);
    }
    if (e->ev_lane_fork) hipEventDestroy(e->ev_lane_fork);
    for (void* p : e->allocs) hipFree(p);
    for (auto& ev : e->ev) if (ev) hipEventDestroy(ev);
    for (auto& pr : e->gemm_ev) { hipEventDestroy(pr.first); hipEventDestroy(pr.second); }
    for (auto& pr : e->attn_ev) { hipEventDestroy(pr.first); hipEventDestroy(pr.second); }
    for (auto& pr : e->layer_ev) { hipEventDestroy(pr.first); hipEventDestroy(pr.second); }
    if (e->tb.gmap) {}
    if (e->bg_stream) { hipStreamSynchronize(e->bg_stream); hipStreamDestroy(e->bg_stream); }
    if (e->full_stream) hipStreamDestroy(e->full_stream);
    for (int i = 0; i < 2; ++i) {
        if (e->side_stream[i]) hipStreamDestroy(e->side_stream[i]);
// ... 11 lines not shown
```

umgen_amd/csrc/frame.h:

```cpp
#pragma once
#include "common.h"

namespace umgen {

constexpr int kPoseBos = 0, kPoseEos = 4, kMapBos = 5, kMapC0 = 6, kMapEos = 1030, kBoxBos = 1031, kBoxC0 = 1032, kBoxEos = 1692,
              kImgBos = 1693, kImgC0 = 1694, kImgEos = 2206;
constexpr int kNMap = 1024, kNBox = 660, kNImg = 512, kNPose = 3;
constexpr int kSlots = 60, kSlotLen = 11, kBoxPad = 1027;
constexpr int kTokPerFrame = kNPose + kNMap + kNBox + kNImg;
constexpr int kOffMap = kNPose, kOffBox = kNPose + kNMap, kOffImg = kNPose + kNMap + kNBox;

enum Stack { STACK_EGO = 0, STACK_MAP = 1, STACK_BOX = 2, STACK_TAR = 3 };
__host__ __device__ inline int stack_len(int st) { return st == STACK_MAP ? 1031 : (st == STACK_BOX ? 1693 : 2207); }

struct EmbedTables {
    const float *egoe, *axe, *be, *tpe, *spe, *tske;
    const bf16_t *fouier_pe, *posi, *grid_posi;
    const float *gmap, *gimg;
    int E;
};

struct WindowTokens {
    const int *pose;
    const int *map;
    const int *box;
    const int *img;
    int B, T;
    int Tfull = 0;
    int t0 = 0;
};

constexpr unsigned kEpochPerStep = 16384;
constexpr int kEngMaxSystolic = 32;

struct SamplerParams {
    int method, top_k, top_k_map, topk_image;
    float p, p_map, temperature;
    int rule_constrain, merge_ar_tar, only_ar;
};

struct OarState {
    int step;
    int frame_idx;
    int use_forced;
    int use_control;
    int done;
    unsigned epoch;
    SamplerParams sp;
};

struct SampleArgs {
    OarState* st;
    EmbedTables tb;
    const float* logits;
    const float* logits_tar;
    int ld_logits;
    int ld_tar;
    int vocab;
    int mod;
    const float* cond;
    float* x_next;
    int* tokens;
    const int* prev_box;
    const unsigned char* control_slot;
    double* boxes;
    int* n_boxes;
    const unsigned long long* seeds;
    const int* forced;
    int* counters;
};

void launch_embed_stack(hipStream_t s, int stack, const EmbedTables& tb, const WindowTokens& w, float* X, float* mapfeat);
void launch_warp_map(hipStream_t s, int stack, const EmbedTables& tb, int B, int T, const float* mapfeat, const float* pose_diff,
                     float* X, float* warped_last, int Tfull = 0, int t0 = 0);
void launch_cond_rows(hipStream_t s, int stack, int B, int T, int E, const float* X, const float* ln_w, const float* warped_last,
                      float* cond);
void launch_first_input(hipStream_t s, int B, int E, const float* tske_row, const float* cond, float* x);
void launch_fixed_token(hipStream_t s, const SampleArgs& a, int B);
void launch_prefix_rows(hipStream_t s, const EmbedTables& tb, const float* tske_row, const float* cond, const int* tokens, int B, int P, float* X,
                        float* x_last);
template <typename T>
void launch_prefix_kv_to_cache(hipStream_t s, const T* qk, const T* vt, int B, int S, int S_pad, int H, int Lmax, T* cache, long scene_stride);
void launch_sample_token(hipStream_t s, const SampleArgs& a, int B);
void launch_sample_rows(hipStream_t s, const float* logits, int V, int k, float temp, const float* u, int* out, int* overflow, int n);
void launch_sample_dbg(hipStream_t s, const float* logits, int V, const SamplerParams& sp, int k, float p, const float* u, int mask_idx, int* out,
                       int* overflow, int n);
void launch_collision_rows(hipStream_t s, const double* boxes, const int* counts, int max_n, int* out, int n_sets);
void launch_sample_ego(hipStream_t s, const float* logits, int vocab, SamplerParams sp, const unsigned long long* seeds, int frame_idx,
                       const int* forced, int* out_tokens, int B, int* overflow);
void launch_ego_queries(hipStream_t s, const EmbedTables& tb, int B, int T, float* x);

}
```

umgen_amd/csrc/frame.hip:

```cpp
#include "bg_queue.h"
#include "frame_body.h"

namespace umgen {

__global__ __launch_bounds__(128) void embed_stack_kernel(int stack, EmbedTables tb, WindowTokens w, float* __restrict__ X,
                                                          float* __restrict__ mapfeat) {
    embed_stack_row(stack, tb, w, X, mapfeat, (long)blockIdx.x, (int)threadIdx.x);
}

__global__ __launch_bounds__(128) void warp_map_kernel(int stack, EmbedTables tb, int T, const float* __restrict__ mapfeat,
                                                       const float* __restrict__ pose_diff, float* __restrict__ X,
                                                       float* __restrict__ warped_last, int Tfull, int t0) {
    warp_map_cell(stack, tb, T, mapfeat, pose_diff, X, warped_last, Tfull, t0, (long)blockIdx.x, (int)threadIdx.x);
}

void launch_embed_stack(hipStream_t s, int stack, const EmbedTables& tb, const WindowTokens& w, float* X, float* mapfeat) {
    const long rows = (long)w.B * w.T * stack_len(stack);
    if (BgRecorder* rec = g_bg_rec) {
        BgOp& o = rec->add(BG_EMBED, 0, (rows + 3) / 4, 128, 60);
        o.h.i0 = stack; o.h.i1 = w.B; o.h.i2 = w.T; o.h.i3 = w.Tfull; o.a.i4 = w.t0; o.a.l1 = rows;
        o.a.p0 = const_cast<int*>(w.pose); o.a.p1 = const_cast<int*>(w.map); o.a.p2 = const_cast<int*>(w.box); o.a.p3 = const_cast<int*>(w.img);
        o.a.p4 = X; o.a.p5 = mapfeat;
        return;
    }
    hipLaunchKernelGGL(embed_stack_kernel, dim3((unsigned)rows), dim3(128), 0, s, stack, tb, w, X, mapfeat);
}


void launch_warp_map(hipStream_t s, int stack, const EmbedTables& tb, int B, int T, const float* mapfeat, const float* pose_diff,
                     float* X, float* warped_last, int Tfull, int t0) {
    if (BgRecorder* rec = g_bg_rec) {
        const long cells = (long)B * T * kNMap;
        BgOp& o = rec->add(BG_WARP, 0, (cells + 3) / 4, 128, 80);
        o.h.i0 = stack; o.h.i1 = T; o.h.i2 = Tfull ? Tfull : T; o.h.i3 = t0; o.a.l1 = cells;
        o.a.p0 = const_cast<float*>(mapfeat); o.a.p1 = const_cast<float*>(pose_diff); o.a.p2 = X; o.a.p3 = warped_last;
        return;
    }
    hipLaunchKernelGGL(warp_map_kernel, dim3((unsigned)((long)B * T * kNMap)), dim3(128), 0, s, stack, tb, T, mapfeat, pose_diff, X,
                       warped_last, Tfull ? Tfull : T, t0);
}

__global__ __launch_bounds__(256) void cond_rows_kernel(int stack, int T, int E, const float* __restrict__ X, const float* __restrict__ ln_w,
                                                        const float* __restrict__ warped_last, float* __restrict__ cond, int n_rows) {
    const int r = blockIdx.x * 4 + (threadIdx.x >> 6);
    const int b = blockIdx.y;
    if (r >= n_rows) return;
    const int lane = threadIdx.x & 63;
    int s;
    if (stack == STACK_MAP) s = kMapBos + r;
    else if (stack == STACK_BOX) s = kBoxBos + r;
    else s = (r < 5) ? r : (kImgBos + (r - 5));
    const int SS = stack_len(stack);
    const float* xr = X + (((long)b * T + (T - 1)) * SS + s) * E;
    float sum = 0.f;
    for (int c = lane; c < E; c += 64) sum += xr[c];
    const float mean = wave_sum(sum) / (float)E;
    float q = 0.f;
    for (int c = lane; c < E; c += 64) { const float d = xr[c] - mean; q += d * d; }
    const float rstd = 1.0f / sqrtf(wave_sum(q) / (float)E + 1e-5f);
    float* o = cond + ((long)b * kSeq + s) * E;
    const float* wl = (stack == STACK_MAP && s >= kMapC0 && s < kMapEos) ? warped_last + ((long)b * kNMap + (s - kMapC0)) * E : nullptr;
    for (int c = lane; c < E; c += 64) {
        float v = (xr[c] - mean) * rstd * ln_w[c];
        if (wl) v += wl[c];
        o[c] = v;
    }
}

void launch_cond_rows(hipStream_t s, int stack, int B, int T, int E, const float* X, const float* ln_w, const float* warped_last,
                      float* cond) {
    const int n_rows = stack == STACK_MAP ? 1026 : (stack == STACK_BOX ? 662 : 5 + 514);
    hipLaunchKernelGGL(cond_rows_kernel, dim3((n_rows + 3) / 4, B), dim3(256), 0, s, stack, T, E, X, ln_w, warped_last, cond, n_rows);
}

__global__ void first_input_kernel(int E, const float* __restrict__ row, const float* __restrict__ cond, float* __restrict__ x) {
    const int b = blockIdx.x;
    for (int c = threadIdx.x; c < E; c += blockDim.x) x[(long)b * E + c] = row[c] + cond[(long)b * kSeq * E + c];
}
void launch_first_input(hipStream_t s, int B, int E, const float* tske_row, const float* cond, float* x) {
    hipLaunchKernelGGL(first_input_kernel, dim3(B), dim3(256), 0, s, E, tske_row, cond, x);
}

__global__ void ego_queries_kernel(EmbedTables tb, int T, float* __restrict__ x) {
    const int j = blockIdx.x % 3;
    const int E = tb.E;
    for (int c = threadIdx.x; c < E; c += blockDim.x)
        x[(long)blockIdx.x * E + c] = (tb.egoe[(long)j * E + c] + tb.spe[(long)j * E + c]) + tb.tpe[(long)(T - 1) * E + c];
}
void launch_ego_queries(hipStream_t s, const EmbedTables& tb, int B, int T, float* x) {
    hipLaunchKernelGGL(ego_queries_kernel, dim3(B * 3), dim3(256), 0, s, tb, T, x);
}

__device__ inline void finish_step(OarState* st) {
    __syncthreads();
    if (gridDim.x == 1) {
        if (threadIdx.x == 0) { st->step += 1; st->epoch += kEpochPerStep; }
        return;
    }
    if (threadIdx.x == 0) {
        const int t = atomicAdd(&st->done, 1);
        if (t == (int)gridDim.x - 1) { st->done = 0; st->step += 1; st->epoch += kEpochPerStep; }
    }
}

constexpr int kMaxKept = 64;
constexpr int kMaxK = 16;
struct SampleShared {
    float cand_v[4 * kMaxK];
    int cand_i[4 * kMaxK];
    float kth;
    int n_kept, n_cand;
    int kept_i[kMaxKept];
    float kept_v[kMaxKept];
    int result;
};

__device__ int block_sample_topk(const float* __restrict__ logits, int V, int k, float temp, float u, int mask_idx, SampleShared& sh, int* overflow) {
    const int tid = threadIdx.x, lane = tid & 63, wave = tid >> 6;
    float v0[32];
#pragma unroll
    for (int i = 0; i < 32; ++i) {
        const int idx = tid + 256 * i;
        v0[i] = (idx < V && idx != mask_idx) ? logits[idx] : -INFINITY;
    }
    const int kk = min(min(k, V), kMaxK);
    if (tid < 4 * kMaxK) { sh.cand_v[tid] = -INFINITY; sh.cand_i[tid] = 0x7fffffff; }
    if (tid == 0) { sh.n_kept = 0; sh.n_cand = 0; }
    __syncthreads();
    {
        float cur = v0[0];
#pragma unroll
        for (int i = 1; i < 32; ++i) cur = fmaxf(cur, v0[i]);
        for (int it = 0; it < kk; ++it) {
            const float wv = wave_max(cur);
            const int first = __ffsll((unsigned long long)__ballot(cur == wv)) - 1;
            if (lane == 0) { sh.cand_v[wave * kMaxK + it] = wv; sh.cand_i[wave * kMaxK + it] = wave * kMaxK + it; }
            if (lane == first) cur = -INFINITY;
        }
    }
    __syncthreads();
    auto rank_candidates = [&](int per_wave) {
        const float cv = sh.cand_v[lane];
        const int ci = sh.cand_i[lane];
        int rank = 0;
        const int ncand = 4 * per_wave;
        for (int jj = 0, w4 = 0, it = 0; jj < ncand; ++jj) {
            const int j = w4 * kMaxK + it;
            const float ov = __int_as_float(__builtin_amdgcn_readlane(__float_as_int(cv), j));
            const int oi = __builtin_amdgcn_readlane(ci, j);
            rank += (ov > cv || (ov == cv && oi < ci)) ? 1 : 0;
            if (++it == per_wave) { it = 0; ++w4; }
        }
        if (rank == kk - 1) sh.kth = cv;
    };
    if (wave == 0) rank_candidates(kk);
    __syncthreads();
    {
        const float T = sh.kth;
#pragma unroll
        for (int i = 0; i < 32; ++i) {
            if (v0[i] >= T && v0[i] > -INFINITY) {
                const int slot = atomicAdd(&sh.n_cand, 1);
                if (slot < kMaxKept) { sh.kept_i[slot] = tid + 256 * i; sh.kept_v[slot] = v0[i]; }
            }
        }
    }
    __syncthreads();
    const int n_cand = sh.n_cand;
    if (n_cand <= kMaxKept) {
        if (wave == 0) {
            const float cv = lane < n_cand ? sh.kept_v[lane] : -INFINITY;
            const int ci = lane < n_cand ? sh.kept_i[lane] : 0x7fffffff;
            int rank = 0;
            for (int j = 0; j < n_cand; ++j) {
                const float ov = __int_as_float(__builtin_amdgcn_readlane(__float_as_int(cv), j));
                const int oi = __builtin_amdgcn_readlane(ci, j);
                rank += (ov > cv || (ov == cv && oi < ci)) ? 1 : 0;
            }
            if (lane < n_cand && rank == kk - 1) sh.kth = cv;
        }
    } else {
        float v[32];
#pragma unroll
        for (int i = 0; i < 32; ++i) v[i] = v0[i];
        if (tid < 4 * kMaxK) { sh.cand_v[tid] = -INFINITY; sh.cand_i[tid] = 0x7fffffff; }
        __syncthreads();
        for (int it = 0; it < kk; ++it) {
            float bv = -INFINITY;
            int bi = 0x7fffffff;
#pragma unroll
            for (int i = 0; i < 32; ++i) {
                const int idx = tid + 256 * i;
                if (v[i] > bv) { bv = v[i]; bi = idx; }
            }
            const float wv = wave_max(bv);
            const int wi = wave_min_i32(bv == wv ? bi : 0x7fffffff);
            if (lane == 0) { sh.cand_v[wave * kMaxK + it] = wv; sh.cand_i[wave * kMaxK + it] = wi; }
            if (bi == wi) {
#pragma unroll
                for (int i = 0; i < 32; ++i)
                    if (tid + 256 * i == wi) v[i] = -INFINITY;
            }
        }
        __syncthreads();
        if (wave == 0) rank_candidates(kk);
    }
    __syncthreads();
    const float kth = sh.kth;
#pragma unroll
    for (int i = 0; i < 32; ++i) {
        const int idx = tid + 256 * i;
        const float l = v0[i];
        if (l >= kth && l > -INFINITY) {
            const int slot = atomicAdd(&sh.n_kept, 1);
            if (slot < kMaxKept) { sh.kept_i[slot] = idx; sh.kept_v[slot] = l; }
        }
    }
    __syncthreads();
    (void)overflow;
    if (sh.n_kept > kMaxKept) {
        if (tid == 0) {
            float zmax = -INFINITY;
            for (int idx = 0; idx < V; ++idx) {
                const float l = idx != mask_idx ? logits[idx] : -INFINITY;
                if (l >= kth && l > -INFINITY) zmax = fmaxf(zmax, l / temp);
            }
            float total = 0.f;
            int last = 0;
            for (int idx = 0; idx < V; ++idx) {
                const float l = idx != mask_idx ? logits[idx] : -INFINITY;
                if (l >= kth && l > -INFINITY) { total = add_rn(total, exp_det(sub_rn(l / temp, zmax))); last = idx; }
            }
            const float target = mul_rn(u, total);
            float c = 0.f;
            int res = last;
            for (int idx = 0; idx < V; ++idx) {
                const float l = idx != mask_idx ? logits[idx] : -INFINITY;
                if (l >= kth && l > -INFINITY) {
                    c = add_rn(c, exp_det(sub_rn(l / temp, zmax)));
                    if (c > target) { res = idx; break; }
                }
            }
            sh.result = res;
        }
    } else if (wave == 0) {
        const int n = min(sh.n_kept, kMaxKept);
        const int ki = lane < n ? sh.kept_i[lane] : 0x7fffffff;
        const float kv = lane < n ? sh.kept_v[lane] : -INFINITY;
        int rank = 0;
        for (int j = 0; j < n; ++j) rank += (__builtin_amdgcn_readlane(ki, j) < ki) ? 1 : 0;
        if (lane < n) { sh.cand_i[rank] = ki; sh.cand_v[rank] = kv; }
        __builtin_amdgcn_wave_barrier();
        const int si = lane < n ? sh.cand_i[lane] : 0;
        const float z = lane < n ? sh.cand_v[lane] / temp : -INFINITY;
        const float zmax = wave_max(z);
        const float ev = lane < n ? exp_det(sub_rn(z, zmax)) : 0.f;
        float total = 0.f;
        for (int a = 0; a < n; ++a) total = add_rn(total, __int_as_float(__builtin_amdgcn_readlane(__float_as_int(ev), a)));
        const float target = mul_rn(u, total);
        float c = 0.f;
        int res = __builtin_amdgcn_readlane(si, n - 1);
        for (int a = 0; a < n; ++a) {
            c = add_rn(c, __int_as_float(__builtin_amdgcn_readlane(__float_as_int(ev), a)));
            if (c > target) { res = __builtin_amdgcn_readlane(si, a); break; }
        }
        if (lane == 0) sh.result = res;
    }
    __syncthreads();
    const int r = sh.result;
    __syncthreads();
    return r;
}

constexpr int kTopPMax = 8192;
struct TopPShared {
    float pr[kTopPMax];
    int ix[kTopPMax];
    float red[4];
    float total;
    int result;
};
__device__ int block_sample_topp(const float* __restrict__ logits, int V, float p, float temp, float u, int mask_idx, TopPShared& sh) {
    const int tid = threadIdx.x, lane = tid & 63, wave = tid >> 6;
    float mx = -INFINITY;
    for (int i = tid; i < kTopPMax; i += 256) {
        const float z = (i < V && i != mask_idx) ? logits[i] / temp : -INFINITY;
        sh.pr[i] = z;
        sh.ix[i] = i;
        mx = fmaxf(mx, z);
    }
    mx = wave_max(mx);
    if (lane == 0) sh.red[wave] = mx;
    __syncthreads();
    mx = fmaxf(fmaxf(sh.red[0], sh.red[1]), fmaxf(sh.red[2], sh.red[3]));
    for (int i = tid; i < kTopPMax; i += 256) sh.pr[i] = exp_det(sub_rn(sh.pr[i], mx));
    __syncthreads();
    if (tid == 0) {
        float t = 0.f;
        for (int i = 0; i < V; ++i) t = add_rn(t, sh.pr[i]);
        sh.total = t;
    }
    __syncthreads();
    const float total = sh.total;
    for (int i = tid; i < kTopPMax; i += 256) sh.pr[i] = (i < V) ? sh.pr[i] / total : -1.f;
    __syncthreads();
    for (int k2 = 2; k2 <= kTopPMax; k2 <<= 1) {
        for (int j = k2 >> 1; j > 0; j >>= 1) {
            for (int i = tid; i < kTopPMax; i += 256) {
                const int l2 = i ^ j;
                if (l2 > i) {
                    const float a = sh.pr[i], b2 = sh.pr[l2];
                    const int ia = sh.ix[i], ib = sh.ix[l2];
                    const bool a_first = (a > b2) || (a == b2 && ia < ib);
                    const bool up = ((i & k2) == 0);
                    if (up ? !a_first : a_first) { sh.pr[i] = b2; sh.pr[l2] = a; sh.ix[i] = ib; sh.ix[l2] = ia; }
                }
            }
            __syncthreads();
        }
    }
    if (tid == 0) {
        float c = 0.f;
        int n = 0;
        while (n < V && !(c > p)) { c = add_rn(c, sh.pr[n]); ++n; }
        float t2 = 0.f;
        for (int i = 0; i < n; ++i) t2 = add_rn(t2, sh.pr[i]);
        const float target = mul_rn(u, t2);
        float cc = 0.f;
        int res = sh.ix[n - 1];
        for (int i = 0; i < n; ++i) {
            cc = add_rn(cc, sh.pr[i]);
            if (cc > target) { res = sh.ix[i]; break; }
        }
        sh.result = res;
    }
    __syncthreads();
    const int r = sh.result;
    __syncthreads();
    return r;
}

union SamplerLds {
    SampleShared k;
    TopPShared p;
};
__device__ inline int block_sample(const SamplerParams& sp, const float* logits, int V, int kparam, float pparam, float u, int mask_idx,
                                   SamplerLds& sh, int* overflow) {
    return sp.method == 0 ? block_sample_topk(logits, V, kparam, sp.temperature, u, mask_idx, sh.k, overflow)
                          : block_sample_topp(logits, V, pparam, sp.temperature, u, mask_idx, sh.p);
}

__device__ inline double box_bin(int i) {
    return (i >= 1023) ? 1.0 : add_rn(mul_rn((double)i, 1.0 / 1023.0), 0.0);
}
// ... 47 lines not shown
                }
            }
        }
    }
    return false;
}

__device__ inline void write_next_input(const SampleArgs& a, int b, int j, const float* emb_f, const bf16_t* emb_b) {
    const int E = a.tb.E;
    const float* cr = a.cond + ((long)b * kSeq + (j + 1)) * E;
    float* xo = a.x_next + (long)b * E;
    for (int c = threadIdx.x; c < E; c += blockDim.x) xo[c] = (emb_f ? emb_f[c] : bf16_to_f32(emb_b[c])) + cr[c];
}
struct CondRow { float v[6]; };
__device__ inline CondRow load_cond_row(const SampleArgs& a, int b, int j) {
    CondRow r;
    const float* cr = a.cond + ((long)b * kSeq + (j + 1)) * a.tb.E;
#pragma unroll
    for (int i = 0; i < 6; ++i) { const int c = threadIdx.x + 256 * i; r.v[i] = c < a.tb.E ? cr[c] : 0.f; }
    return r;
}
__device__ inline void write_next_input(const SampleArgs& a, int b, const float* emb_f, const CondRow& r) {
    float* xo = a.x_next + (long)b * a.tb.E;
#pragma unroll
    for (int i = 0; i < 6; ++i) { const int c = threadIdx.x + 256 * i; if (c < a.tb.E) xo[c] = emb_f[c] + r.v[i]; }
}

__global__ __launch_bounds__(256) void fixed_token_kernel(SampleArgs a) {
    const int b = blockIdx.x, j = a.st->step, E = a.tb.E;
    const int aux = fixed_aux_id(j);
    const int* toks = a.tokens + (long)b * kTokPerFrame;
    if (aux >= 0) write_next_input(a, b, j, a.tb.axe + (long)aux * E, nullptr);
    else if (j < kPoseEos) write_next_input(a, b, j, nullptr, a.tb.fouier_pe + (long)toks[j - 1] * E);
    else if (j < kMapEos) write_next_input(a, b, j, a.tb.gmap + (long)toks[kOffMap + (j - kMapC0)] * E, nullptr);
    else write_next_input(a, b, j, a.tb.be + (long)toks[kOffBox + (j - kBoxC0)] * E, nullptr);
    finish_step(a.st);
}
void launch_fixed_token(hipStream_t s, const SampleArgs& a, int B) { hipLaunchKernelGGL(fixed_token_kernel, dim3(B), dim3(256), 0, s, a); }

__global__ __launch_bounds__(256) void prefix_rows_kernel(EmbedTables tb, const float* __restrict__ tske_row, const float* __restrict__ cond,
                                                          const int* __restrict__ tokens, int P, float* __restrict__ X, float* __restrict__ x_last) {
    const int b = blockIdx.x / P, j = blockIdx.x % P, E = tb.E;
    const float* cr = cond + ((long)b * kSeq + j) * E;
    float* xo = j + 1 < P ? X + ((long)b * (P - 1) + j) * E : x_last + (long)b * E;
    const int* toks = tokens + (long)b * kTokPerFrame;
    const float* ef = nullptr;
    const bf16_t* eb = nullptr;
    if (j == 0) ef = tske_row;
    else {
        const int jp = j - 1, aux = fixed_aux_id(jp);
        if (aux >= 0) ef = tb.axe + (long)aux * E;
        else if (jp < kPoseEos) eb = tb.fouier_pe + (long)toks[jp - 1] * E;
        else if (jp < kMapEos) ef = tb.gmap + (long)toks[kOffMap + (jp - kMapC0)] * E;
        else ef = tb.be + (long)toks[kOffBox + (jp - kBoxC0)] * E;
    }
    for (int c = threadIdx.x; c < E; c += blockDim.x) xo[c] = (ef ? ef[c] : bf16_to_f32(eb[c])) + cr[c];
}
void launch_prefix_rows(hipStream_t s, const EmbedTables& tb, const float* tske_row, const float* cond, const int* tokens, int B, int P, float* X,
                        float* x_last) {
    hipLaunchKernelGGL(prefix_rows_kernel, dim3(B * P), dim3(256), 0, s, tb, tske_row, cond, tokens, P, X, x_last);
}

template <typename T>
__global__ __launch_bounds__(256) void prefix_kv_to_cache_kernel(const T* __restrict__ qk, const T* __restrict__ vt, int S, int S_pad, int H, int Lmax,
                                                                  T* __restrict__ cache, long scene_stride) {
    const int E = H * kHeadDim;
    const int b = blockIdx.y;
    const long i = (long)blockIdx.x * 256 + threadIdx.x;
    if (i >= (long)S * E) return;
    const int j = (int)(i / E), hd = (int)(i % E), h = hd / kHeadDim, d = hd % kHeadDim;
    T* c = cache + (long)b * scene_stride;
    c[((long)h * Lmax + j) * kHeadDim + d] = qk[((long)b * S + j) * 2 * E + E + hd];
    c[((long)(H + h) * Lmax + j) * kHeadDim + d] = vt[(((long)b * H + h) * kHeadDim + d) * S_pad + j];
}
template <typename T>
void launch_prefix_kv_to_cache(hipStream_t s, const T* qk, const T* vt, int B, int S, int S_pad, int H, int Lmax, T* cache, long scene_stride) {
    const long n = (long)S * H * kHeadDim;
    hipLaunchKernelGGL(prefix_kv_to_cache_kernel<T>, dim3((unsigned)((n + 255) / 256), B), dim3(256), 0, s, qk, vt, S, S_pad, H, Lmax, cache, scene_stride);
}
template void launch_prefix_kv_to_cache<float>(hipStream_t, const float*, const float*, int, int, int, int, int, float*, long);
template void launch_prefix_kv_to_cache<bf16_t>(hipStream_t, const bf16_t*, const bf16_t*, int, int, int, int, int, bf16_t*, long);
template void launch_prefix_kv_to_cache<f16_t>(hipStream_t, const f16_t*, const f16_t*, int, int, int, int, int, f16_t*, long);

__global__ __launch_bounds__(256) void sample_token_kernel(SampleArgs a) {
    __shared__ SamplerLds sh;
    __shared__ float cor[64][8];
    __shared__ int s_tok;
    const int b = blockIdx.x, j = a.st->step, frame = a.st->frame_idx, E = a.tb.E;
    const SamplerParams sp = a.st->sp;
    const bool use_forced = a.st->use_forced != 0, use_control = a.st->use_control != 0;
    const int pos1 = j + 1;
    const unsigned long long seed = a.seeds[b];
    const CondRow crow = load_cond_row(a, b, j);
    const float* lg = a.logits + (long)b * a.ld_logits;
    const int topk = a.mod == 1 ? sp.top_k_map : (a.mod == 3 ? sp.topk_image : sp.top_k);
    const float topp = a.mod == 1 ? sp.p_map : (a.mod == 3 ? (float)sp.topk_image : sp.p);
    int tok = block_sample(sp, lg, a.vocab, topk, topp, rng_uniform(seed, frame, pos1, DRAW_MAIN), -1, sh, a.counters + 7);
    int off, k;
    if (a.mod == 1) { off = kOffMap; k = j - kMapC0; }
    else if (a.mod == 2) { off = kOffBox; k = j - kBoxC0; }
    else { off = kOffImg; k = j - kImgC0; }
    int* toks = a.tokens + (long)b * kTokPerFrame;
    if (a.mod == 2) {
        const float* lt = a.logits_tar + ((long)b * kNBox + k) * a.ld_tar;
        const int prev = a.prev_box[(long)b * kNBox + k];
        if (use_control) {
            const int object_id = (pos1 - 1032) / kSlotLen;
            if (object_id < kSlots && a.control_slot[b * kSlots + object_id]) {
                tok = block_sample(sp, lt, a.vocab, sp.top_k, sp.p, rng_uniform(seed, frame, pos1, DRAW_CONTROL), a.vocab - 1, sh, a.counters + 7);
                if (threadIdx.x == 0) atomicAdd(a.counters + 1, 1);
            }
        }
        if (tok == kBoxPad && sp.merge_ar_tar && prev != kBoxPad && !sp.only_ar) {
            tok = block_sample(sp, lt, a.vocab, sp.top_k, sp.p, rng_uniform(seed, frame, pos1, DRAW_PAD_AVOID), -1, sh, a.counters + 7);
            if (threadIdx.x == 0) atomicAdd(a.counters + 0, 1);
        }
        if (sp.rule_constrain && !use_forced && tok != kBoxPad && (pos1 - 1032) % kSlotLen == 0) {
            if (threadIdx.x == 0) {
                double* boxes = a.boxes + (long)b * 64 * 10;
                int n = a.n_boxes[b];
                if (n == 0) {
                    const double ego[10] = {0, 0, 0, 5.176, 2.297, 1.777, 0, 0, 0, 0};
                    for (int q = 0; q < 10; ++q) boxes[q] = ego[q];
                    n = 1;
                }
                double* nb = boxes + n * 10;
                for (int q = 0; q < 10; ++q) {
                    const int t = toks[off + k - 10 + q];
                    const int right = min(max(t, 0), 1023), left = min(max(t - 1, 0), 1023);
                    const double v = add_rn(box_bin(left), box_bin(right)) / 2.0;
                    nb[q] = add_rn(mul_rn(v, kBoxHi[q] - kBoxLo[q]), kBoxLo[q]);
                }
                ++n;
                const bool collision = check_collision_dev(boxes, n, cor);
                const bool newborn = (prev == kBoxPad);
                atomicAdd(a.counters + 2, 1);
                if (collision) atomicAdd(a.counters + 3, 1);
                int t2 = tok;
                if ((newborn && collision) || (n > 30 && newborn)) {
                    for (int q = 1; q <= 10; ++q) toks[off + k - q] = kBoxPad;
                    --n;
                    t2 = kBoxPad;
                    atomicAdd(a.counters + 4, 1);
                }
                a.n_boxes[b] = n;
                s_tok = t2;
            }
            __syncthreads();
            tok = s_tok;
        }
    }
    if (use_forced) {
        const int ft = a.forced[(long)b * kTokPerFrame + off + k];
        if (threadIdx.x == 0 && ft != tok) atomicAdd(a.counters + 5, 1);
        tok = ft;
    }
    if (threadIdx.x == 0) toks[off + k] = tok;
    const float* emb = (a.mod == 1) ? a.tb.gmap + (long)tok * E : (a.mod == 3 ? a.tb.gimg + (long)tok * E : a.tb.be + (long)tok * E);
    write_next_input(a, b, emb, crow);
    finish_step(a.st);
}
void launch_sample_token(hipStream_t s, const SampleArgs& a, int B) { hipLaunchKernelGGL(sample_token_kernel, dim3(B), dim3(256), 0, s, a); }

__global__ __launch_bounds__(256) void sample_ego_kernel(const float* __restrict__ logits, int vocab, SamplerParams sp,
                                                         const unsigned long long* __restrict__ seeds, int frame_idx,
                                                         const int* __restrict__ forced, int* __restrict__ out_tokens, int* overflow) {
    __shared__ SamplerLds sh;
    const int b = blockIdx.x / 3, jq = blockIdx.x % 3;
    int tok = block_sample(sp, logits + (long)blockIdx.x * vocab, vocab, sp.top_k, sp.p,
                           rng_uniform(seeds[b], frame_idx, kSeq + jq, DRAW_MAIN), -1, sh, overflow);
    if (forced) tok = forced[(long)b * kTokPerFrame + jq];
    if (threadIdx.x == 0) out_tokens[b * 3 + jq] = tok;
}
void launch_sample_ego(hipStream_t s, const float* logits, int vocab, SamplerParams sp, const unsigned long long* seeds, int frame_idx,
                       const int* forced, int* out_tokens, int B, int* overflow) {
    hipLaunchKernelGGL(sample_ego_kernel, dim3(B * 3), dim3(256), 0, s, logits, vocab, sp, seeds, frame_idx, forced, out_tokens, overflow);
}

__global__ __launch_bounds__(256) void sample_rows_kernel(const float* __restrict__ logits, int V, int k, float temp, const float* __restrict__ u,
                                                          int* __restrict__ out, int* overflow) {
    __shared__ SamplerLds sh;
    const int tok = block_sample_topk(logits + (long)blockIdx.x * V, V, k, temp, u[blockIdx.x], -1, sh.k, overflow);
    if (threadIdx.x == 0) out[blockIdx.x] = tok;
}
void launch_sample_rows(hipStream_t s, const float* logits, int V, int k, float temp, const float* u, int* out, int* overflow, int n) {
    hipLaunchKernelGGL(sample_rows_kernel, dim3(n), dim3(256), 0, s, logits, V, k, temp, u, out, overflow);
}

__global__ __launch_bounds__(256) void sample_dbg_kernel(const float* __restrict__ logits, int V, SamplerParams sp, int k, float p,
                                                         const float* __restrict__ u, int mask_idx, int* __restrict__ out, int* overflow) {
    __shared__ SamplerLds sh;
    const int tok = block_sample(sp, logits + (long)blockIdx.x * V, V, k, p, u[blockIdx.x], mask_idx, sh, overflow);
    if (threadIdx.x == 0) out[blockIdx.x] = tok;
}
void launch_sample_dbg(hipStream_t s, const float* logits, int V, const SamplerParams& sp, int k, float p, const float* u, int mask_idx, int* out,
                       int* overflow, int n) {
    hipLaunchKernelGGL(sample_dbg_kernel, dim3(n), dim3(256), 0, s, logits, V, sp, k, p, u, mask_idx, out, overflow);
}

__global__ __launch_bounds__(64) void collision_rows_kernel(const double* __restrict__ boxes, const int* __restrict__ counts, int max_n,
                                                            int* __restrict__ out) {
    __shared__ float cor[64][8];
    if (threadIdx.x == 0) out[blockIdx.x] = check_collision_dev(boxes + (long)blockIdx.x * max_n * 10, counts[blockIdx.x], cor) ? 1 : 0;
}
void launch_collision_rows(hipStream_t s, const double* boxes, const int* counts, int max_n, int* out, int n_sets) {
    hipLaunchKernelGGL(collision_rows_kernel, dim3(n_sets), dim3(64), 0, s, boxes, counts, max_n, out);
}

}
```

umgen_amd/csrc/gemv.hip:

```cpp
#include "kernels.h"

namespace umgen {

template <typename T> struct WChunk;
template <> struct WChunk<bf16_t> { uint4 v; };
template <> struct WChunk<f16_t> { uint4 v; };
template <> struct WChunk<float> { float4 a, b; };

typedef unsigned int u32x4_t __attribute__((ext_vector_type(4)));
typedef float f32x4v_t __attribute__((ext_vector_type(4)));
template <bool NT = true>
__device__ inline void wload(WChunk<bf16_t>& w, const bf16_t* p) {
#ifndef UMGEN_NO_NT
    if (NT) {
        const u32x4_t t = __builtin_nontemporal_load(reinterpret_cast<const u32x4_t*>(p));
        w.v = make_uint4(t.x, t.y, t.z, t.w);
        return;
    }
#endif
    w.v = *reinterpret_cast<const uint4*>(p);
}
template <bool NT = true>
__device__ inline void wload(WChunk<f16_t>& w, const f16_t* p) {
    WChunk<bf16_t> t;
    wload<NT>(t, reinterpret_cast<const bf16_t*>(p));
    w.v = t.v;
}
template <bool NT = true>
__device__ inline void wload(WChunk<float>& w, const float* p) {
#ifndef UMGEN_NO_NT
    if (NT) {
        const f32x4v_t a = __builtin_nontemporal_load(reinterpret_cast<const f32x4v_t*>(p));
        const f32x4v_t b = __builtin_nontemporal_load(reinterpret_cast<const f32x4v_t*>(p + 4));
        w.a = make_float4(a.x, a.y, a.z, a.w);
        w.b = make_float4(b.x, b.y, b.z, b.w);
        return;
    }
#endif
    w.a = *reinterpret_cast<const float4*>(p);
    w.b = *reinterpret_cast<const float4*>(p + 4);
}

__device__ inline void tile_row_of_block(int bid, int rows, int& tile, int& row) {
    const int q = bid >> 3;
    row = q % rows;
    tile = (q / rows) * 8 + (bid & 7);
}
inline int tile_row_grid(int tiles, int rows) { return ((tiles + 7) / 8) * 8 * rows; }
__device__ inline void wzero(WChunk<bf16_t>& w) { w.v = make_uint4(0, 0, 0, 0); }
__device__ inline void wzero(WChunk<f16_t>& w) { w.v = make_uint4(0, 0, 0, 0); }
__device__ inline void wzero(WChunk<float>& w) { w.a = make_float4(0, 0, 0, 0); w.b = w.a; }
__device__ inline void wunpack(const WChunk<bf16_t>& w, float (&o)[8]) {
    o[0] = __uint_as_float(w.v.x << 16); o[1] = __uint_as_float(w.v.x & 0xffff0000u);
    o[2] = __uint_as_float(w.v.y << 16); o[3] = __uint_as_float(w.v.y & 0xffff0000u);
    o[4] = __uint_as_float(w.v.z << 16); o[5] = __uint_as_float(w.v.z & 0xffff0000u);
    o[6] = __uint_as_float(w.v.w << 16); o[7] = __uint_as_float(w.v.w & 0xffff0000u);
}
__device__ inline void wunpack(const WChunk<f16_t>& w, float (&o)[8]) {
    const f16x8_t h = __builtin_bit_cast(f16x8_t, w.v);
#pragma unroll
    for (int e = 0; e < 8; ++e) o[e] = (float)h[e];
}
__device__ inline void wunpack(const WChunk<float>& w, float (&o)[8]) {
    o[0] = w.a.x; o[1] = w.a.y; o[2] = w.a.z; o[3] = w.a.w; o[4] = w.b.x; o[5] = w.b.y; o[6] = w.b.z; o[7] = w.b.w;
}

template <typename T, int MB, int NCH, int RPW, bool PERROW = false>
__device__ __forceinline__ void gemv_ln_body(const GemvArgs& a, int bid) {
    const int lane = threadIdx.x & 63, wave = threadIdx.x >> 6;
    const int K = a.K;
    const T* W = reinterpret_cast<const T*>(a.W);
    int tile = bid, mb = 0;
    if (PERROW) { tile_row_of_block(bid, (a.M + MB - 1) / MB, tile, mb); mb *= MB; }
    const int Mloc = PERROW ? min(MB, a.M - mb) : a.M;
    const int n0 = (tile * 4 + wave) * RPW;
    if (n0 >= a.N) return;
    WChunk<T> w[RPW][NCH];
#pragma unroll
    for (int r = 0; r < RPW; ++r) {
        const T* wr = W + (long)min(n0 + r, a.N - 1) * K;
#pragma unroll
        for (int i = 0; i < NCH; ++i) {
            const int c = lane * 8 + 512 * i;
            if (c < K) wload<!PERROW>(w[r][i], wr + c); else wzero(w[r][i]);
        }
    }
    float bias[RPW];
#pragma unroll
    for (int r = 0; r < RPW; ++r) bias[r] = (a.bias && n0 + r < a.N) ? a.bias[n0 + r] : 0.f;
    const int pos = a.d_len ? *a.d_len : 0;
    const float* xbase = a.x + (a.d_xoff ? (long)(*a.d_xoff) * a.xoff_mul : 0L);
    float lw[NCH][8];
    if (a.ln_w) {
#pragma unroll
        for (int i = 0; i < NCH; ++i) {
            const int c = lane * 8 + 512 * i;
            if (c < K) load8(a.ln_w + c, lw[i]);
        }
    }
    for (int m0 = 0; m0 < Mloc; m0 += MB) {
        float xv[MB][NCH][8];
#pragma unroll
        for (int m = 0; m < MB; ++m) {
            const float* xr = xbase + (long)(mb + min(m0 + m, Mloc - 1)) * a.ldx;
#pragma unroll
            for (int i = 0; i < NCH; ++i) {
                const int c = lane * 8 + 512 * i;
                if (c < K) load8(xr + c, xv[m][i]);
                else {
#pragma unroll
                    for (int e = 0; e < 8; ++e) xv[m][i][e] = 0.f;
                }
            }
        }
        if (a.ln_w) {
#pragma unroll
            for (int m = 0; m < MB; ++m) {
                float s = 0.f;
#pragma unroll
                for (int i = 0; i < NCH; ++i)
#pragma unroll
                    for (int e = 0; e < 8; ++e) s += xv[m][i][e];
                const float mean = wave_sum(s) / (float)K;
                float q = 0.f;
#pragma unroll
                for (int i = 0; i < NCH; ++i) {
                    if (lane * 8 + 512 * i < K) {
#pragma unroll
                        for (int e = 0; e < 8; ++e) { const float d = xv[m][i][e] - mean; q += d * d; }
                    }
                }
                const float rstd = 1.0f / sqrtf(wave_sum(q) / (float)K + 1e-5f);
#pragma unroll
                for (int i = 0; i < NCH; ++i) {
                    if (lane * 8 + 512 * i < K) {
#pragma unroll
                        for (int e = 0; e < 8; ++e) xv[m][i][e] = (xv[m][i][e] - mean) * rstd * lw[i][e];
                    }
                }
            }
        }
#pragma unroll
        for (int r = 0; r < RPW; ++r) {
            float acc[MB];
#pragma unroll
            for (int m = 0; m < MB; ++m) acc[m] = 0.f;
#pragma unroll
            for (int i = 0; i < NCH; ++i) {
                float w8[8];
                wunpack(w[r][i], w8);
#pragma unroll
                for (int m = 0; m < MB; ++m)
#pragma unroll
                    for (int e = 0; e < 8; ++e) acc[m] = fmaf(w8[e], xv[m][i][e], acc[m]);
            }
#pragma unroll
            for (int m = 0; m < MB; ++m) acc[m] = wave_sum(acc[m]);
            const int n = n0 + r;
            if (lane == 0 && n < a.N) {
#pragma unroll
                for (int m = 0; m < MB; ++m) {
                    const int mm = mb + m0 + m;
                    if (m0 + m < Mloc) {
                        const float v = acc[m] + bias[r];
                        if (a.out_mode == GEMV_OUT_QKV) {
                            if (n < a.E) __builtin_nontemporal_store(v, &a.out[(long)mm * a.ldo + n]);
                            else {
                                const int c = n - a.E, kvsel = c / a.E, hc = c % a.E;
                                const long H = a.E / kHeadDim;
                                reinterpret_cast<T*>(a.cache)[(long)mm * a.scene_stride + ((kvsel * H + hc / kHeadDim) * a.Lmax + pos) * kHeadDim +
                                                              hc % kHeadDim] = Cvt<T>::from_f(v);
                            }
                        } else {
                            if (a.out_mode == GEMV_OUT_GELU) __builtin_nontemporal_store(gelu_erf(v), &a.out[(long)mm * a.ldo + n]);
                            else a.out[(long)mm * a.ldo + n] = v;
                        }
                    }
                }
            }
        }
    }
}

template <typename T, int MB, int NCH, int RPW, bool PERROW = false>
__global__ __launch_bounds__(256) void gemv_ln_kernel(GemvArgs a) {
#ifdef UMGEN_DRY_DECODE
    return;
#endif
    gemv_ln_body<T, MB, NCH, RPW, PERROW>(a, blockIdx.x);
}

template <typename T, int NCH>
static void launch_gemv_nch(hipStream_t s, const GemvArgs& a) {
    constexpr int RPW = 2;
    const int grid = (a.N + 4 * RPW - 1) / (4 * RPW);
    if (a.M > 1 && a.rows_per_block == 1)
        hipLaunchKernelGGL((gemv_ln_kernel<T, 1, NCH, RPW, true>), dim3(tile_row_grid(grid, a.M)), dim3(256), 0, s, a);
    else if (a.M > 2 && a.rows_per_block == 2)
        hipLaunchKernelGGL((gemv_ln_kernel<T, 2, NCH, RPW, true>), dim3(tile_row_grid(grid, (a.M + 1) / 2)), dim3(256), 0, s, a);
    else if (a.M == 1) hipLaunchKernelGGL((gemv_ln_kernel<T, 1, NCH, RPW>), dim3(grid), dim3(256), 0, s, a);
    else if (a.M == 2) hipLaunchKernelGGL((gemv_ln_kernel<T, 2, NCH, RPW>), dim3(grid), dim3(256), 0, s, a);
    else hipLaunchKernelGGL((gemv_ln_kernel<T, 4, NCH, RPW>), dim3(grid), dim3(256), 0, s, a);
}

template <typename T>
void launch_gemv(hipStream_t s, const GemvArgs& a) {
    if (a.K <= 512) launch_gemv_nch<T, 1>(s, a);
    else if (a.K <= 1024) launch_gemv_nch<T, 2>(s, a);
    else launch_gemv_nch<T, 3>(s, a);
}
template void launch_gemv<float>(hipStream_t, const GemvArgs&);
template void launch_gemv<bf16_t>(hipStream_t, const GemvArgs&);
template void launch_gemv<f16_t>(hipStream_t, const GemvArgs&);


template <typename T, int MB, int NCH, bool COMBINE, bool PERROW = false>
__global__ __launch_bounds__(256) void gemv_resid_kernel(GemvResidArgs a_in) {
#ifdef UMGEN_DRY_DECODE
    return;
#endif
    extern __shared__ __attribute__((aligned(16))) float as[];
    const int lane = threadIdx.x & 63, wave = threadIdx.x >> 6;
    GemvResidArgs a = a_in;
    int tile = blockIdx.x;
    if (PERROW) {
        int mb;
        tile_row_of_block(blockIdx.x, (a_in.M + MB - 1) / MB, tile, mb);
        mb *= MB;
        a.M = min(MB, a_in.M - mb);
        a.x += (long)mb * a.ldx;
        if (a.a) a.a += (long)mb * a.lda;
        if (a.part) a.part += (long)mb * a.H * kAttnRec;
    }
    const int K = a.K;
    const T* W = reinterpret_cast<const T*>(a.W);
    const int n = tile * 4 + wave;
    const bool active = n < a.N;
    WChunk<T> w[NCH];
    {
        const T* wr = W + (long)min(n, a.N - 1) * K;
#pragma unroll
        for (int i = 0; i < NCH; ++i) {
            const int c = lane * 8 + 512 * i;
            if (c < K) wload<!PERROW>(w[i], wr + c); else wzero(w[i]);
        }
    }
    const float bias = (a.bias && active) ? a.bias[n] : 0.f;
    if (COMBINE) {
        float* s_w = as + (long)a.M * K;
        const int ns = a.ns;
        const int tid = threadIdx.x;
        const int n_el = a.M * K;
        float4 ov[3][kAttnPad / 4];
        auto load_chunk = [&](int base) {
#pragma unroll
            for (int it = 0; it < 3; ++it) {
                const int e = base + tid + 256 * it;
                if (e < n_el) {
                    const int m = e / K, col = e % K;
                    const float4* po = reinterpret_cast<const float4*>(a.part + (long)(m * a.H + col / kHeadDim) * kAttnRec + 2 * kAttnPad +
                                                                       (col % kHeadDim) * kAttnPad);
#pragma unroll
                    for (int i = 0; i < kAttnPad / 4; ++i) ov[it][i] = (4 * i < ns) ? po[i] : make_float4(0.f, 0.f, 0.f, 0.f);
                }
            }
// ... 289 lines not shown
```

umgen_amd/csrc/kernels.h:

```cpp
#pragma once
#include "common.h"

namespace umgen {

enum GemmMode {
    GEMM_STORE = 0,
    GEMM_RESID = 1,
    GEMM_STORE_F32 = 2,
    GEMM_VT = 3
};
struct GemmArgs {
    const void* P; const void* Q;
    int Mi, Nj, K;
    long ldp, ldq;
    long strideP, strideQ;
    int batch;
    int mode;
    const float* bias;
    int gelu;
    void* out;
    long ldo;
    long strideO;
    int H;
    int tile256;
};
bool gemm256_supported(const GemmArgs& a);
hipError_t gemm256_prepare();
int gemm256_read_stamps(unsigned long long* out16);
template <typename TT> void launch_gemm256(hipStream_t s, const GemmArgs& a);
void record_gemm256(const GemmArgs& a);
template <typename TT> void launch_gemm_mfma(hipStream_t s, const GemmArgs& a);
template <typename TP, typename TQ> void launch_gemm_valu(hipStream_t s, const GemmArgs& a);

template <typename T> void launch_layernorm(hipStream_t s, const float* x, long row_stride, long n_rows, int E, const float* w, T* out);

template <typename TT> void launch_attn_spatial_mfma(hipStream_t s, const TT* qk, const TT* vt, TT* y, int F, int S, int S_pad, int H);
template <typename T> void launch_attn_spatial_valu(hipStream_t s, const T* qk, const T* vt, T* y, int F, int S, int S_pad, int H);
void launch_attn_spatial_f32_mfma(hipStream_t s, const float* qk, const float* vt, float* y, int F, int S, int S_pad, int H);
template <typename TT> void launch_attn_causal_mfma(hipStream_t s, const TT* qk, const TT* vt, TT* y, int F, int S, int S_pad, int H);
void launch_attn_causal_f32(hipStream_t s, const float* qk, const float* vt, float* y, int F, int S, int S_pad, int H);
struct TemporalRange { int t0; void* cache; int Tcap; int write; int q0 = 0; };
template <typename T> void launch_attn_temporal(hipStream_t s, const T* qkv, T* y, int B, int Tn, int S, int H,
                                                TemporalRange tr = TemporalRange{0, nullptr, 0, 0});

constexpr int kAttnSplit = 18;
constexpr int kAttnChunk = 128;
inline int attn_nsplit(int L) { return L <= 0 ? 1 : (L + kAttnChunk - 1) / kAttnChunk; }
constexpr int kAttnPad = 20;
constexpr int kAttnRec = 2 * kAttnPad + kHeadDim * kAttnPad;
template <typename T> void launch_attn_partial(hipStream_t s, const float* q, const T* kv_base, long scene_stride, long head_stride,
                                               long key_stride, long v_off, int NQ, int q_per_scene, int H, const int* d_len, int len_add,
                                               int ns, float* part);

enum GemvOut {
    GEMV_OUT_F32 = 0,
    GEMV_OUT_GELU = 1,
    GEMV_OUT_QKV = 2
};
struct GemvArgs {
    const float* x; long ldx;
    const int* d_xoff; long xoff_mul;
    const float* ln_w;
    const void* W; const float* bias; int N, K, M;
    int out_mode;
    float* out; long ldo;
    void* cache; long scene_stride; const int* d_len; int Lmax;
    int rows_per_block;
    int E;
};
template <typename T> void launch_gemv(hipStream_t s, const GemvArgs& a);

struct GemvResidArgs {
    const float* a; long lda; const float* part; int H;
    int ns;
    const void* W; const float* bias; int N, K, M;
    float* x; long ldx;
    int rows_per_block;
};
template <typename T> void launch_gemv_resid(hipStream_t s, const GemvResidArgs& a);

struct DecodeLayerArgs {
    const float *ln_a, *bqkv, *bo, *ln_b;
    const void *Wqkv, *Wo, *Wfc, *Wproj;
    float* x;
    float *q, *h, *part;
    void* cache; long scene_stride; int Lmax; const int* d_len;
    int B, E, H, ns, rows_per_block;
};
template <typename T> void launch_decode_layer(hipStream_t s, const DecodeLayerArgs& a);

inline int ego_cross_nsplit() { return attn_nsplit(kSeq); }
inline void launch_ego_self_attn(hipStream_t s, const float* q, const float* qkv3, int M, int H, float* part) {
    const int E = H * kHeadDim;
    launch_attn_partial<float>(s, q, qkv3 + E, 3L * 3 * E, kHeadDim, 3L * E, E, M, 3, H, nullptr, 3, 1, part);
}
template <typename T>
void launch_ego_cross_attn(hipStream_t s, const float* q, const T* kv, int M, int H, float* part) {
    const int E = H * kHeadDim;
    launch_attn_partial<T>(s, q, kv, (long)kSeq * 2 * E, kHeadDim, 2L * E, E, M, 3, H, nullptr, kSeq, ego_cross_nsplit(), part);
}

enum RowsMode {
    ROWS_F32 = 0,
    ROWS_GELU = 1,
    ROWS_QKV = 2,
    ROWS_RESID = 3
};
constexpr int kRowsMaxM = 64;
constexpr int kRowsMaxNB = 4;
__host__ __device__ inline long frag_index(int m, int k) {
    return ((((long)(k >> 5) * kRowsMaxNB + (m >> 4)) * 64 + ((k & 31) >> 3) * 16 + (m & 15)) << 3) + (k & 7);
}
struct RowsArgs {
    const float* x; int M;
    const float* ln_w;
    const void* W; const float* bias; int N, K;
    int mode;
    float* out; long ldo;
    float* out_frag;
    void* cache; long scene_stride; const int* d_len; int Lmax; int E;
};
template <typename TT> void launch_rows_mfma(hipStream_t s, const RowsArgs& a);
void launch_rows_to_frag(hipStream_t s, const float* x, long ldx, int M, int K, float* xf);
template <typename TT> void launch_attn_decode_batched(hipStream_t s, const float* q, const TT* cache, long scene_stride, int B, int H, int Lmax,
                                                        const int* d_len, float* y);

constexpr int kEngE = 768, kEngH = 16;
#ifndef UMGEN_ENG_MFMA
#define UMGEN_ENG_MFMA 12
#endif
constexpr int kEngThreads = 512;
constexpr int kEngGroup = 32;
constexpr int kEngWpUnits = 18;
constexpr int kEngLocStride = 3 * kEngE + 2 * kEngH * 50 + kEngE + kEngGroup * kEngE + kEngE;
struct OarLayerDev {
    const bf16_t *Wqkv, *Wo, *Wfc, *Wproj;
    const bf16_t *Wp2;
    const float *bqkv, *bo, *ln_a, *ln_b;
    const bf16_t *Wf2;
};
struct OarState;
struct BgQueue;
struct OarEngineArgs {
    const OarLayerDev* layers; int n_layers;
    bf16_t* kvcache; long kv_layer_stride, kv_scene_stride; int Lmax;
    bf16_t* vtcache; long vt_layer_stride, vt_scene_stride;
    float* xdec;
    const OarState* st;
    unsigned long long* gx;
    unsigned long long* gloc;
    unsigned int* ticket;
// ... 43 lines not shown
```

Measured before the change: 1972 scene-tokens/s.

## Fuse output-head GEMV and token sampling into one spin-synchronized kernel

For single-scene decoding on the engine path, the LayerNorm+head GEMV and the top-k/top-p sampling are launched as one kernel. Worker blocks compute logits and publish each value into an epoch-tagged 64-bit granule. Block 0 computes its own slice, spins until every vocab entry carries the current tag, then samples in registers and writes the next input. This removes one kernel launch and the gap between launches on every decode step, at the cost of an inter-block spin wait that depends on all blocks being co-resident, plus extra atomic traffic.

```diff
diff --git a/umgen_amd/_lib.py b/umgen_amd/_lib.py
--- a/umgen_amd/_lib.py
+++ b/umgen_amd/_lib.py
@@ -17,7 +17,7 @@
            "umgen_dbg_rows", "umgen_dbg_attn_decode_batched", "umgen_dbg_sample", "umgen_dbg_collision",
            "umgen_dbg_gemv_modes", "umgen_dbg_gemv_resid", "umgen_dbg_attn_partial", "umgen_dbg_decode_layer"]
 
-HEADERS = ("common.h", "kernels.h", "frame.h", "oar_common.h", "bg_queue.h", "bg_worker.h", "gemm256_body.h", "attn_body.h", "rowops_body.h", "frame_body.h")
+HEADERS = ("common.h", "kernels.h", "frame.h", "oar_common.h", "bg_queue.h", "bg_worker.h", "gemm256_body.h", "attn_body.h", "rowops_body.h", "frame_body.h", "gemv_body.h")
 
 PREC_FP32, PREC_BF16, PREC_FP16 = 0, 1, 2
 DT_F32, DT_BF16, DT_F16, DT_F64 = 0, 1, 2, 3
diff --git a/umgen_amd/csrc/engine.hip b/umgen_amd/csrc/engine.hip
--- a/umgen_amd/csrc/engine.hip
+++ b/umgen_amd/csrc/engine.hip
@@ -137,6 +137,11 @@
     void* burn_buf = nullptr;
     int fg_xcds = 8;
     unsigned eng_epoch = 16u;
+    bool tail_on = true;
+    unsigned long long* tail_gran = nullptr;
+    bool tail_fused(int B) const {
+        return tail_on && tail_gran && tsz == 2 && B == 1 && !in_lanes && !use_batched(B) && !use_wide(B) && eng_for(stream) && E > 512 && E <= 1024;
+    }
     int step_graph_NG = -1;
     bool in_capture = false;
     const EngStream* eng_for(hipStream_t s) const {
@@ -706,6 +711,8 @@
     return v;
 }
 
+inline int64_t tail_kernels(const umgen_engine* e, int B, int mod) { return mod == 0 ? 1 : (mod == 2 ? 3 : 2) - (e->tail_fused(B) ? 1 : 0); }
+
 template <typename T>
 int enqueue_step(umgen_engine* e, int B, int mod, int ns, const umgen_trace* tr, int j) {
     const int E = e->E;
@@ -740,8 +747,17 @@
         const void* head = mod == 1 ? e->head_ar_map : (mod == 2 ? e->head_ar_box : e->head_ar_img);
         const int V = mod == 1 ? e->cfg.map_vocab : (mod == 2 ? e->cfg.bbox3d_vocab : e->cfg.img_vocab);
         bool head_done = false;
+        const bool fused = e->tail_fused(B);
+        sa.mod = mod;
+        sa.vocab = V;
         if constexpr (sizeof(T) == 2) {
-            if (e->use_batched(B)) {
+            if (fused) {
+                GemvArgs g{};
+                g.x = e->xdec; g.ldx = E; g.ln_w = e->ln_oar; g.W = head; g.N = V; g.K = E; g.M = 1; g.out_mode = GEMV_OUT_F32; g.out = e->logits;
+                g.ldo = sa.ld_logits; g.E = E; g.gran = e->tail_gran; g.d_tag = &e->d_state->epoch;
+                launch_head_sample<T>(st, g, sa, e->eng_err);
+                head_done = true;
+            } else if (e->use_batched(B)) {
                 RowsArgs r{};
                 r.x = e->xfrag; r.M = B; r.ln_w = e->ln_oar; r.W = head; r.N = V; r.K = E; r.mode = ROWS_F32; r.out = e->logits; r.ldo = sa.ld_logits; r.E = E;
                 launch_rows_mfma<T>(e->stream, r);
@@ -754,9 +770,7 @@
             const int k = mod == 1 ? j - kMapC0 : (mod == 2 ? j - kBoxC0 : j - kImgC0);
             if (dst) HIPCHK(e, hipMemcpyAsync(dst + (size_t)k * V, e->logits, (size_t)V * 4, hipMemcpyDeviceToHost, st));
         }
-        sa.mod = mod;
-        sa.vocab = V;
-        launch_sample_token(st, sa, B);
+        if (!fused) launch_sample_token(st, sa, B);
     }
     return 0;
 }
@@ -941,6 +955,7 @@
         HIPCHK(e, hipDeviceSynchronize());
         HIPCHK(e, hipMemset(e->eng_gx, 0, (size_t)e->cfg.max_batch * kEngE * 8));
         HIPCHK(e, hipMemset(e->eng_gloc, 0, e->eng_gloc_bytes));
+        HIPCHK(e, hipMemset(e->tail_gran, 0, (size_t)8192 * 8));
         e->eng_epoch = 16u;
     }
     OarState s0{j_begin, io.frame_idx, forced ? 1 : 0, io.control_slot ? 1 : 0, 0, e->eng_epoch, sp};
@@ -1143,12 +1158,12 @@
                 HIPCHK(e, hipGraphDestroy(g));
             }
             HIPCHK(e, hipGraphLaunch(ge, st));
-            e->tm.oar_kernels += (int64_t)(run - 1) * ((eng ? (wide ? B : 1) : 5 * (int64_t)e->oar.size()) + (mod == 0 ? 1 : (mod == 2 ? 3 : 2)));
+            e->tm.oar_kernels += (int64_t)(run - 1) * ((eng ? (wide ? B : 1) : 5 * (int64_t)e->oar.size()) + tail_kernels(e, B, mod));
             j += run - 1;
         } else if (int rc = enqueue_step<T>(e, B, mod, ns, tr, j)) {
             return rc;
         }
-        e->tm.oar_kernels += (eng ? (wide ? B : 1) : 5 * (int64_t)e->oar.size()) + (mod == 0 ? 1 : (mod == 2 ? 3 : 2));
+        e->tm.oar_kernels += (eng ? (wide ? B : 1) : 5 * (int64_t)e->oar.size()) + tail_kernels(e, B, mod);
     }
     e->tm.oar_steps += steps_run;
     const bool drained = e->bg_engine && e->bg_pending;
@@ -1514,6 +1529,8 @@
     const char* be_env = getenv("UMGEN_BG_ENGINE");
     e->bg_engine = e->eng_enabled && cfg->max_batch == 1 && cfg->max_cond_frames >= 2 && cfg->max_cond_frames <= 32 && !ov_env && !(be_env && be_env[0] == '0');
     if (e->bg_engine) { e->overlap = true; e->overlap_mode = 1; }
+    const char* tail_env = getenv("UMGEN_ENGINE_TAIL");
+    e->tail_on = !(tail_env && tail_env[0] == '0');
     int bg_cus = 64;
     if (const char* bc = getenv("UMGEN_BG_CUS")) bg_cus = std::max(32, std::min(128, atoi(bc)));
     if (e->bg_engine) {
@@ -1754,6 +1771,8 @@
         if (int rc = dev_alloc(e, reinterpret_cast<void**>(&e->eng_gloc), e->eng_gloc_bytes)) return rc;
         if (int rc = dalloc(e, &e->eng_ticket, (size_t)16)) return rc;
         if (int rc = dalloc(e, &e->eng_err, (size_t)4)) return rc;
+        if (int rc = dalloc(e, &e->tail_gran, (size_t)8192)) return rc;
+        HIPCHK(e, hipMemset(e->tail_gran, 0, (size_t)8192 * 8));
         HIPCHK(e, hipMemset(e->eng_ticket, 0, 64));
         if (getenv("UMGEN_DEBUG_TIMING") && !e->bg_engine) {
             if (int rc = dalloc(e, &e->eng_stamps, (size_t)16)) return rc;
@@ -2106,6 +2125,7 @@
         if (e->eng_enabled) {
             HIPCHK(e, hipMemset(e->eng_gx, 0, (size_t)e->cfg.max_batch * kEngE * 8));
             HIPCHK(e, hipMemset(e->eng_gloc, 0, e->eng_gloc_bytes));
+            HIPCHK(e, hipMemset(e->tail_gran, 0, (size_t)8192 * 8));
         }
         if (e->wide_enabled) HIPCHK(e, hipMemset(e->wide_gran, 0, oar_engine_wide_granules() * 8));
         e->eng_epoch = 16u;
diff --git a/umgen_amd/csrc/frame.h b/umgen_amd/csrc/frame.h
--- a/umgen_amd/csrc/frame.h
+++ b/umgen_amd/csrc/frame.h
@@ -82,6 +82,9 @@
 template <typename T>
 void launch_prefix_kv_to_cache(hipStream_t s, const T* qk, const T* vt, int B, int S, int S_pad, int H, int Lmax, T* cache, long scene_stride);
 void launch_sample_token(hipStream_t s, const SampleArgs& a, int B);
+struct GemvArgs;
+template <typename T>
+void launch_head_sample(hipStream_t s, const GemvArgs& g, const SampleArgs& a, unsigned* err);
 void launch_sample_rows(hipStream_t s, const float* logits, int V, int k, float temp, const float* u, int* out, int* overflow, int n);
 void launch_sample_dbg(hipStream_t s, const float* logits, int V, const SamplerParams& sp, int k, float p, const float* u, int mask_idx, int* out,
                        int* overflow, int n);
diff --git a/umgen_amd/csrc/frame.hip b/umgen_amd/csrc/frame.hip
--- a/umgen_amd/csrc/frame.hip
+++ b/umgen_amd/csrc/frame.hip
@@ -1,5 +1,6 @@
 #include "bg_queue.h"
 #include "frame_body.h"
+#include "gemv_body.h"
 
 namespace umgen {
 
@@ -91,9 +92,9 @@
     hipLaunchKernelGGL(ego_queries_kernel, dim3(B * 3), dim3(256), 0, s, tb, T, x);
 }
 
-__device__ inline void finish_step(OarState* st) {
-    __syncthreads();
-    if (gridDim.x == 1) {
+__device__ inline void finish_step(OarState* st, bool single = false) {
+    __syncthreads();
+    if (single || gridDim.x == 1) {
         if (threadIdx.x == 0) { st->step += 1; st->epoch += kEpochPerStep; }
         return;
     }
@@ -115,14 +116,10 @@
     int result;
 };
 
-__device__ int block_sample_topk(const float* __restrict__ logits, int V, int k, float temp, float u, int mask_idx, SampleShared& sh, int* overflow) {
+template <bool PUBLISH = false>
+__device__ __forceinline__ int block_sample_topk_v(const float (&v0)[32], const float* __restrict__ logits, int V, int k, float temp, float u, int mask_idx,
+                                                   SampleShared& sh, int* overflow) {
     const int tid = threadIdx.x, lane = tid & 63, wave = tid >> 6;
-    float v0[32];
-#pragma unroll
-    for (int i = 0; i < 32; ++i) {
-        const int idx = tid + 256 * i;
-        v0[i] = (idx < V && idx != mask_idx) ? logits[idx] : -INFINITY;
-    }
     const int kk = min(min(k, V), kMaxK);
     if (tid < 4 * kMaxK) { sh.cand_v[tid] = -INFINITY; sh.cand_i[tid] = 0x7fffffff; }
     if (tid == 0) { sh.n_kept = 0; sh.n_cand = 0; }
@@ -219,6 +216,12 @@
     __syncthreads();
     (void)overflow;
     if (sh.n_kept > kMaxKept) {
+        if (PUBLISH) {
+#pragma unroll
+            for (int i = 0; i < 32; ++i)
+                if (tid + 256 * i < V) const_cast<float*>(logits)[tid + 256 * i] = v0[i];
+            __syncthreads();
+        }
         if (tid == 0) {
             float zmax = -INFINITY;
             for (int idx = 0; idx < V; ++idx) {
@@ -270,6 +273,15 @@
     const int r = sh.result;
     __syncthreads();
     return r;
+}
+__device__ int block_sample_topk(const float* __restrict__ logits, int V, int k, float temp, float u, int mask_idx, SampleShared& sh, int* overflow) {
+    float v0[32];
+#pragma unroll
+    for (int i = 0; i < 32; ++i) {
+        const int idx = threadIdx.x + 256 * i;
+        v0[i] = (idx < V && idx != mask_idx) ? logits[idx] : -INFINITY;
+    }
+    return block_sample_topk_v(v0, logits, V, k, temp, u, mask_idx, sh, overflow);
 }
 
 constexpr int kTopPMax = 8192;
@@ -483,20 +495,19 @@
 template void launch_prefix_kv_to_cache<bf16_t>(hipStream_t, const bf16_t*, const bf16_t*, int, int, int, int, int, bf16_t*, long);
 template void launch_prefix_kv_to_cache<f16_t>(hipStream_t, const f16_t*, const f16_t*, int, int, int, int, int, f16_t*, long);
 
-__global__ __launch_bounds__(256) void sample_token_kernel(SampleArgs a) {
+template <bool SINGLE, typename MainDraw>
+__device__ __forceinline__ void sample_token_body(const SampleArgs& a, int b, int j, const CondRow& crow, MainDraw main_draw) {
     __shared__ SamplerLds sh;
     __shared__ float cor[64][8];
     __shared__ int s_tok;
-    const int b = blockIdx.x, j = a.st->step, frame = a.st->frame_idx, E = a.tb.E;
+    const int frame = a.st->frame_idx, E = a.tb.E;
     const SamplerParams sp = a.st->sp;
     const bool use_forced = a.st->use_forced != 0, use_control = a.st->use_control != 0;
     const int pos1 = j + 1;
     const unsigned long long seed = a.seeds[b];
-    const CondRow crow = load_cond_row(a, b, j);
-    const float* lg = a.logits + (long)b * a.ld_logits;
     const int topk = a.mod == 1 ? sp.top_k_map : (a.mod == 3 ? sp.topk_image : sp.top_k);
     const float topp = a.mod == 1 ? sp.p_map : (a.mod == 3 ? (float)sp.topk_image : sp.p);
-    int tok = block_sample(sp, lg, a.vocab, topk, topp, rng_uniform(seed, frame, pos1, DRAW_MAIN), -1, sh, a.counters + 7);
+    int tok = main_draw(sp, topk, topp, rng_uniform(seed, frame, pos1, DRAW_MAIN), sh);
     int off, k;
     if (a.mod == 1) { off = kOffMap; k = j - kMapC0; }
     else if (a.mod == 2) { off = kOffBox; k = j - kBoxC0; }
@@ -559,9 +570,71 @@
     if (threadIdx.x == 0) toks[off + k] = tok;
     const float* emb = (a.mod == 1) ? a.tb.gmap + (long)tok * E : (a.mod == 3 ? a.tb.gimg + (long)tok * E : a.tb.be + (long)tok * E);
     write_next_input(a, b, emb, crow);
-    finish_step(a.st);
+    finish_step(a.st, SINGLE);
+}
+
+__global__ __launch_bounds__(256) void sample_token_kernel(SampleArgs a) {
+    const int b = blockIdx.x, j = a.st->step;
+    const CondRow crow = load_cond_row(a, b, j);
+    const float* lg = a.logits + (long)b * a.ld_logits;
+    sample_token_body<false>(a, b, j, crow, [&](const SamplerParams& sp, int topk, float topp, float u, SamplerLds& sh) {
+        return block_sample(sp, lg, a.vocab, topk, topp, u, -1, sh, a.counters + 7);
+    });
 }
 void launch_sample_token(hipStream_t s, const SampleArgs& a, int B) { hipLaunchKernelGGL(sample_token_kernel, dim3(B), dim3(256), 0, s, a); }
+
+constexpr unsigned kTailSpinLimit = 2000000u;
+constexpr int kTailRPW = 4;
+template <typename T>
+__global__ __launch_bounds__(256) void head_sample_kernel(GemvArgs g, SampleArgs a, unsigned* err) {
+    if (blockIdx.x != 0) {
+        gemv_ln_body<T, 1, 2, kTailRPW>(g, blockIdx.x);
+        return;
+    }
+    const int tid = threadIdx.x, j = a.st->step, V = a.vocab;
+    const unsigned tag = a.st->epoch;
+    const CondRow crow = load_cond_row(a, 0, j);
+    gemv_ln_body<T, 1, 2, kTailRPW>(g, 0);
+    float v0[32];
+    unsigned need = 0u;
+#pragma unroll
+    for (int i = 0; i < 32; ++i) {
+        v0[i] = -INFINITY;
+        if (tid + 256 * i < V) need |= 1u << i;
+    }
+    for (unsigned spins = 0;;) {
+        unsigned long long x[32];
+#pragma unroll
+        for (int i = 0; i < 32; ++i) x[i] = __hip_atomic_load(g.gran + min(tid + 256 * i, V - 1), __ATOMIC_RELAXED, __HIP_MEMORY_SCOPE_AGENT);
+#pragma unroll
+        for (int i = 0; i < 32; ++i)
+            if (((need >> i) & 1u) && (unsigned)(x[i] >> 32) == tag) {
+                v0[i] = __uint_as_float((unsigned)x[i]);
+                need &= ~(1u << i);
+            }
+        if (!__syncthreads_or(need != 0u)) break;
+        if (++spins > kTailSpinLimit || ((spins & 255u) == 0 && __hip_atomic_load(err, __ATOMIC_RELAXED, __HIP_MEMORY_SCOPE_AGENT))) {
+            if (tid == 0) atomicCAS(err, 0u, tag | 0x80000000u);
+            break;
+        }
+        __builtin_amdgcn_s_sleep(1);
+    }
+    float* lg = const_cast<float*>(a.logits);
+    sample_token_body<true>(a, 0, j, crow, [&](const SamplerParams& sp, int topk, float topp, float u, SamplerLds& sh) {
+        if (sp.method == 0) return block_sample_topk_v<true>(v0, lg, V, topk, sp.temperature, u, -1, sh.k, a.counters + 7);
+#pragma unroll
+        for (int i = 0; i < 32; ++i)
+            if (tid + 256 * i < V) lg[tid + 256 * i] = v0[i];
+        __syncthreads();
+        return block_sample_topp(lg, V, topp, sp.temperature, u, -1, sh.p);
+    });
+}
+template <typename T>
+void launch_head_sample(hipStream_t s, const GemvArgs& g, const SampleArgs& a, unsigned* err) {
+    hipLaunchKernelGGL(head_sample_kernel<T>, dim3((g.N + 4 * kTailRPW - 1) / (4 * kTailRPW)), dim3(256), 0, s, g, a, err);
+}
+template void launch_head_sample<bf16_t>(hipStream_t, const GemvArgs&, const SampleArgs&, unsigned*);
+template void launch_head_sample<f16_t>(hipStream_t, const GemvArgs&, const SampleArgs&, unsigned*);
 
 __global__ __launch_bounds__(256) void sample_ego_kernel(const float* __restrict__ logits, int vocab, SamplerParams sp,
                                                          const unsigned long long* __restrict__ seeds, int frame_idx,
diff --git a/umgen_amd/csrc/gemv.hip b/umgen_amd/csrc/gemv.hip
--- a/umgen_amd/csrc/gemv.hip
+++ b/umgen_amd/csrc/gemv.hip
@@ -1,186 +1,7 @@
-#include "kernels.h"
+#include "gemv_body.h"
 
 namespace umgen {
 
-template <typename T> struct WChunk;
-template <> struct WChunk<bf16_t> { uint4 v; };
-template <> struct WChunk<f16_t> { uint4 v; };
-template <> struct WChunk<float> { float4 a, b; };
-
-typedef unsigned int u32x4_t __attribute__((ext_vector_type(4)));
-typedef float f32x4v_t __attribute__((ext_vector_type(4)));
-template <bool NT = true>
-__device__ inline void wload(WChunk<bf16_t>& w, const bf16_t* p) {
-#ifndef UMGEN_NO_NT
-    if (NT) {
-        const u32x4_t t = __builtin_nontemporal_load(reinterpret_cast<const u32x4_t*>(p));
-        w.v = make_uint4(t.x, t.y, t.z, t.w);
-        return;
-    }
-#endif
-    w.v = *reinterpret_cast<const uint4*>(p);
-}
-template <bool NT = true>
-__device__ inline void wload(WChunk<f16_t>& w, const f16_t* p) {
-    WChunk<bf16_t> t;
-    wload<NT>(t, reinterpret_cast<const bf16_t*>(p));
-    w.v = t.v;
-}
-template <bool NT = true>
-__device__ inline void wload(WChunk<float>& w, const float* p) {
-#ifndef UMGEN_NO_NT
-    if (NT) {
-        const f32x4v_t a = __builtin_nontemporal_load(reinterpret_cast<const f32x4v_t*>(p));
-        const f32x4v_t b = __builtin_nontemporal_load(reinterpret_cast<const f32x4v_t*>(p + 4));
-        w.a = make_float4(a.x, a.y, a.z, a.w);
-        w.b = make_float4(b.x, b.y, b.z, b.w);
-        return;
-    }
-#endif
-    w.a = *reinterpret_cast<const float4*>(p);
-    w.b = *reinterpret_cast<const float4*>(p + 4);
-}
-
-__device__ inline void tile_row_of_block(int bid, int rows, int& tile, int& row) {
-    const int q = bid >> 3;
-    row = q % rows;
-    tile = (q / rows) * 8 + (bid & 7);
-}
-inline int tile_row_grid(int tiles, int rows) { return ((tiles + 7) / 8) * 8 * rows; }
-__device__ inline void wzero(WChunk<bf16_t>& w) { w.v = make_uint4(0, 0, 0, 0); }
-__device__ inline void wzero(WChunk<f16_t>& w) { w.v = make_uint4(0, 0, 0, 0); }
-__device__ inline void wzero(WChunk<float>& w) { w.a = make_float4(0, 0, 0, 0); w.b = w.a; }
-__device__ inline void wunpack(const WChunk<bf16_t>& w, float (&o)[8]) {
-    o[0] = __uint_as_float(w.v.x << 16); o[1] = __uint_as_float(w.v.x & 0xffff0000u);
-    o[2] = __uint_as_float(w.v.y << 16); o[3] = __uint_as_float(w.v.y & 0xffff0000u);
-    o[4] = __uint_as_float(w.v.z << 16); o[5] = __uint_as_float(w.v.z & 0xffff0000u);
-    o[6] = __uint_as_float(w.v.w << 16); o[7] = __uint_as_float(w.v.w & 0xffff0000u);
-}
-__device__ inline void wunpack(const WChunk<f16_t>& w, float (&o)[8]) {
-    const f16x8_t h = __builtin_bit_cast(f16x8_t, w.v);
-#pragma unroll
-    for (int e = 0; e < 8; ++e) o[e] = (float)h[e];
-}
-__device__ inline void wunpack(const WChunk<float>& w, float (&o)[8]) {
-    o[0] = w.a.x; o[1] = w.a.y; o[2] = w.a.z; o[3] = w.a.w; o[4] = w.b.x; o[5] = w.b.y; o[6] = w.b.z; o[7] = w.b.w;
-}
-
-template <typename T, int MB, int NCH, int RPW, bool PERROW = false>
-__device__ __forceinline__ void gemv_ln_body(const GemvArgs& a, int bid) {
-    const int lane = threadIdx.x & 63, wave = threadIdx.x >> 6;
-    const int K = a.K;
-    const T* W = reinterpret_cast<const T*>(a.W);
-    int tile = bid, mb = 0;
-    if (PERROW) { tile_row_of_block(bid, (a.M + MB - 1) / MB, tile, mb); mb *= MB; }
-    const int Mloc = PERROW ? min(MB, a.M - mb) : a.M;
-    const int n0 = (tile * 4 + wave) * RPW;
-    if (n0 >= a.N) return;
-    WChunk<T> w[RPW][NCH];
-#pragma unroll
-    for (int r = 0; r < RPW; ++r) {
-        const T* wr = W + (long)min(n0 + r, a.N - 1) * K;
-#pragma unroll
-        for (int i = 0; i < NCH; ++i) {
-            const int c = lane * 8 + 512 * i;
-            if (c < K) wload<!PERROW>(w[r][i], wr + c); else wzero(w[r][i]);
-        }
-    }
-    float bias[RPW];
-#pragma unroll
-    for (int r = 0; r < RPW; ++r) bias[r] = (a.bias && n0 + r < a.N) ? a.bias[n0 + r] : 0.f;
-    const int pos = a.d_len ? *a.d_len : 0;
-    const float* xbase = a.x + (a.d_xoff ? (long)(*a.d_xoff) * a.xoff_mul : 0L);
-    float lw[NCH][8];
-    if (a.ln_w) {
-#pragma unroll
-        for (int i = 0; i < NCH; ++i) {
-            const int c = lane * 8 + 512 * i;
-            if (c < K) load8(a.ln_w + c, lw[i]);
-        }
-    }
-    for (int m0 = 0; m0 < Mloc; m0 += MB) {
-        float xv[MB][NCH][8];
-#pragma unroll
-        for (int m = 0; m < MB; ++m) {
-            const float* xr = xbase + (long)(mb + min(m0 + m, Mloc - 1)) * a.ldx;
-#pragma unroll
-            for (int i = 0; i < NCH; ++i) {
-                const int c = lane * 8 + 512 * i;
-                if (c < K) load8(xr + c, xv[m][i]);
-                else {
-#pragma unroll
-                    for (int e = 0; e < 8; ++e) xv[m][i][e] = 0.f;
-                }
-            }
-        }
-        if (a.ln_w) {
-#pragma unroll
-            for (int m = 0; m < MB; ++m) {
-                float s = 0.f;
-#pragma unroll
-                for (int i = 0; i < NCH; ++i)
-#pragma unroll
-                    for (int e = 0; e < 8; ++e) s += xv[m][i][e];
-                const float mean = wave_sum(s) / (float)K;
-                float q = 0.f;
-#pragma unroll
-                for (int i = 0; i < NCH; ++i) {
-                    if (lane * 8 + 512 * i < K) {
-#pragma unroll
-                        for (int e = 0; e < 8; ++e) { const float d = xv[m][i][e] - mean; q += d * d; }
-                    }
-                }
-                const float rstd = 1.0f / sqrtf(wave_sum(q) / (float)K + 1e-5f);
-#pragma unroll
-                for (int i = 0; i < NCH; ++i) {
-                    if (lane * 8 + 512 * i < K) {
-#pragma unroll
-                        for (int e = 0; e < 8; ++e) xv[m][i][e] = (xv[m][i][e] - mean) * rstd * lw[i][e];
-                    }
-                }
-            }
-        }
-#pragma unroll
-        for (int r = 0; r < RPW; ++r) {
-            float acc[MB];
-#pragma unroll
-            for (int m = 0; m < MB; ++m) acc[m] = 0.f;
-#pragma unroll
-            for (int i = 0; i < NCH; ++i) {
-                float w8[8];
-                wunpack(w[r][i], w8);
-#pragma unroll
-                for (int m = 0; m < MB; ++m)
-#pragma unroll
-                    for (int e = 0; e < 8; ++e) acc[m] = fmaf(w8[e], xv[m][i][e], acc[m]);
-            }
-#pragma unroll
-            for (int m = 0; m < MB; ++m) acc[m] = wave_sum(acc[m]);
-            const int n = n0 + r;
-            if (lane == 0 && n < a.N) {
-#pragma unroll
-                for (int m = 0; m < MB; ++m) {
-                    const int mm = mb + m0 + m;
-                    if (m0 + m < Mloc) {
-                        const float v = acc[m] + bias[r];
-                        if (a.out_mode == GEMV_OUT_QKV) {
-                            if (n < a.E) __builtin_nontemporal_store(v, &a.out[(long)mm * a.ldo + n]);
-                            else {
-                                const int c = n - a.E, kvsel = c / a.E, hc = c % a.E;
-                                const long H = a.E / kHeadDim;
-                                reinterpret_cast<T*>(a.cache)[(long)mm * a.scene_stride + ((kvsel * H + hc / kHeadDim) * a.Lmax + pos) * kHeadDim +
-                                                              hc % kHeadDim] = Cvt<T>::from_f(v);
-                            }
-                        } else {
-                            if (a.out_mode == GEMV_OUT_GELU) __builtin_nontemporal_store(gelu_erf(v), &a.out[(long)mm * a.ldo + n]);
-                            else a.out[(long)mm * a.ldo + n] = v;
-                        }
-                    }
-                }
-            }
-        }
-    }
-}
 
 template <typename T, int MB, int NCH, int RPW, bool PERROW = false>
 __global__ __launch_bounds__(256) void gemv_ln_kernel(GemvArgs a) {
diff --git a/umgen_amd/csrc/gemv_body.h b/umgen_amd/csrc/gemv_body.h
--- /dev/null
+++ b/umgen_amd/csrc/gemv_body.h
@@ -0,0 +1,190 @@
+#pragma once
+#include "kernels.h"
+
+namespace umgen {
+
+template <typename T> struct WChunk;
+template <> struct WChunk<bf16_t> { uint4 v; };
+template <> struct WChunk<f16_t> { uint4 v; };
+template <> struct WChunk<float> { float4 a, b; };
+
+typedef unsigned int u32x4_t __attribute__((ext_vector_type(4)));
+typedef float f32x4v_t __attribute__((ext_vector_type(4)));
+template <bool NT = true>
+__device__ inline void wload(WChunk<bf16_t>& w, const bf16_t* p) {
+#ifndef UMGEN_NO_NT
+    if (NT) {
+        const u32x4_t t = __builtin_nontemporal_load(reinterpret_cast<const u32x4_t*>(p));
+        w.v = make_uint4(t.x, t.y, t.z, t.w);
+        return;
+    }
+#endif
+    w.v = *reinterpret_cast<const uint4*>(p);
+}
+template <bool NT = true>
+__device__ inline void wload(WChunk<f16_t>& w, const f16_t* p) {
+    WChunk<bf16_t> t;
+    wload<NT>(t, reinterpret_cast<const bf16_t*>(p));
+    w.v = t.v;
+}
+template <bool NT = true>
+__device__ inline void wload(WChunk<float>& w, const float* p) {
+#ifndef UMGEN_NO_NT
+    if (NT) {
+        const f32x4v_t a = __builtin_nontemporal_load(reinterpret_cast<const f32x4v_t*>(p));
+        const f32x4v_t b = __builtin_nontemporal_load(reinterpret_cast<const f32x4v_t*>(p + 4));
+        w.a = make_float4(a.x, a.y, a.z, a.w);
+        w.b = make_float4(b.x, b.y, b.z, b.w);
+        return;
+    }
+#endif
+    w.a = *reinterpret_cast<const float4*>(p);
+    w.b = *reinterpret_cast<const float4*>(p + 4);
+}
+
+__device__ inline void tile_row_of_block(int bid, int rows, int& tile, int& row) {
+    const int q = bid >> 3;
+    row = q % rows;
+    tile = (q / rows) * 8 + (bid & 7);
+}
+inline int tile_row_grid(int tiles, int rows) { return ((tiles + 7) / 8) * 8 * rows; }
+__device__ inline void wzero(WChunk<bf16_t>& w) { w.v = make_uint4(0, 0, 0, 0); }
+__device__ inline void wzero(WChunk<f16_t>& w) { w.v = make_uint4(0, 0, 0, 0); }
+__device__ inline void wzero(WChunk<float>& w) { w.a = make_float4(0, 0, 0, 0); w.b = w.a; }
+__device__ inline void wunpack(const WChunk<bf16_t>& w, float (&o)[8]) {
+    o[0] = __uint_as_float(w.v.x << 16); o[1] = __uint_as_float(w.v.x & 0xffff0000u);
+    o[2] = __uint_as_float(w.v.y << 16); o[3] = __uint_as_float(w.v.y & 0xffff0000u);
+    o[4] = __uint_as_float(w.v.z << 16); o[5] = __uint_as_float(w.v.z & 0xffff0000u);
+    o[6] = __uint_as_float(w.v.w << 16); o[7] = __uint_as_float(w.v.w & 0xffff0000u);
+}
+__device__ inline void wunpack(const WChunk<f16_t>& w, float (&o)[8]) {
+    const f16x8_t h = __builtin_bit_cast(f16x8_t, w.v);
+#pragma unroll
+    for (int e = 0; e < 8; ++e) o[e] = (float)h[e];
+}
+__device__ inline void wunpack(const WChunk<float>& w, float (&o)[8]) {
+    o[0] = w.a.x; o[1] = w.a.y; o[2] = w.a.z; o[3] = w.a.w; o[4] = w.b.x; o[5] = w.b.y; o[6] = w.b.z; o[7] = w.b.w;
+}
+
+template <typename T, int MB, int NCH, int RPW, bool PERROW = false>
+__device__ __forceinline__ void gemv_ln_body(const GemvArgs& a, int bid) {
+    const int lane = threadIdx.x & 63, wave = threadIdx.x >> 6;
+    const int K = a.K;
+    const T* W = reinterpret_cast<const T*>(a.W);
+    int tile = bid, mb = 0;
+    if (PERROW) { tile_row_of_block(bid, (a.M + MB - 1) / MB, tile, mb); mb *= MB; }
+    const int Mloc = PERROW ? min(MB, a.M - mb) : a.M;
+    const int n0 = (tile * 4 + wave) * RPW;
+    if (n0 >= a.N) return;
+    WChunk<T> w[RPW][NCH];
+#pragma unroll
+    for (int r = 0; r < RPW; ++r) {
+        const T* wr = W + (long)min(n0 + r, a.N - 1) * K;
+#pragma unroll
+        for (int i = 0; i < NCH; ++i) {
+            const int c = lane * 8 + 512 * i;
+            if (c < K) wload<!PERROW>(w[r][i], wr + c); else wzero(w[r][i]);
+        }
+    }
+    float bias[RPW];
+#pragma unroll
+    for (int r = 0; r < RPW; ++r) bias[r] = (a.bias && n0 + r < a.N) ? a.bias[n0 + r] : 0.f;
+    const int pos = a.d_len ? *a.d_len : 0;
+    const unsigned gtag = a.gran ? *a.d_tag : 0u;
+    const float* xbase = a.x + (a.d_xoff ? (long)(*a.d_xoff) * a.xoff_mul : 0L);
+    float lw[NCH][8];
+    if (a.ln_w) {
+#pragma unroll
+        for (int i = 0; i < NCH; ++i) {
+            const int c = lane * 8 + 512 * i;
+            if (c < K) load8(a.ln_w + c, lw[i]);
+        }
+    }
+    for (int m0 = 0; m0 < Mloc; m0 += MB) {
+        float xv[MB][NCH][8];
+#pragma unroll
+        for (int m = 0; m < MB; ++m) {
+            const float* xr = xbase + (long)(mb + min(m0 + m, Mloc - 1)) * a.ldx;
+#pragma unroll
+            for (int i = 0; i < NCH; ++i) {
+                const int c = lane * 8 + 512 * i;
+                if (c < K) load8(xr + c, xv[m][i]);
+                else {
+#pragma unroll
+                    for (int e = 0; e < 8; ++e) xv[m][i][e] = 0.f;
+                }
+            }
+        }
+        if (a.ln_w) {
+#pragma unroll
+            for (int m = 0; m < MB; ++m) {
+                float s = 0.f;
+#pragma unroll
+                for (int i = 0; i < NCH; ++i)
+#pragma unroll
+                    for (int e = 0; e < 8; ++e) s += xv[m][i][e];
+                const float mean = wave_sum(s) / (float)K;
+                float q = 0.f;
+#pragma unroll
+                for (int i = 0; i < NCH; ++i) {
+                    if (lane * 8 + 512 * i < K) {
+#pragma unroll
+                        for (int e = 0; e < 8; ++e) { const float d = xv[m][i][e] - mean; q += d * d; }
+                    }
+                }
+                const float rstd = 1.0f / sqrtf(wave_sum(q) / (float)K + 1e-5f);
+#pragma unroll
+                for (int i = 0; i < NCH; ++i) {
+                    if (lane * 8 + 512 * i < K) {
+#pragma unroll
+                        for (int e = 0; e < 8; ++e) xv[m][i][e] = (xv[m][i][e] - mean) * rstd * lw[i][e];
+                    }
+                }
+            }
+        }
+#pragma unroll
+        for (int r = 0; r < RPW; ++r) {
+            float acc[MB];
+#pragma unroll
+            for (int m = 0; m < MB; ++m) acc[m] = 0.f;
+#pragma unroll
+            for (int i = 0; i < NCH; ++i) {
+                float w8[8];
+                wunpack(w[r][i], w8);
+#pragma unroll
+                for (int m = 0; m < MB; ++m)
+#pragma unroll
+                    for (int e = 0; e < 8; ++e) acc[m] = fmaf(w8[e], xv[m][i][e], acc[m]);
+            }
+#pragma unroll
+            for (int m = 0; m < MB; ++m) acc[m] = wave_sum(acc[m]);
+            const int n = n0 + r;
+            if (lane == 0 && n < a.N) {
+#pragma unroll
+                for (int m = 0; m < MB; ++m) {
+                    const int mm = mb + m0 + m;
+                    if (m0 + m < Mloc) {
+                        const float v = acc[m] + bias[r];
+                        if (a.out_mode == GEMV_OUT_QKV) {
+                            if (n < a.E) __builtin_nontemporal_store(v, &a.out[(long)mm * a.ldo + n]);
+                            else {
+                                const int c = n - a.E, kvsel = c / a.E, hc = c % a.E;
+                                const long H = a.E / kHeadDim;
+                                reinterpret_cast<T*>(a.cache)[(long)mm * a.scene_stride + ((kvsel * H + hc / kHeadDim) * a.Lmax + pos) * kHeadDim +
+                                                              hc % kHeadDim] = Cvt<T>::from_f(v);
+                            }
+                        } else {
+                            if (a.out_mode == GEMV_OUT_GELU) __builtin_nontemporal_store(gelu_erf(v), &a.out[(long)mm * a.ldo + n]);
+                            else a.out[(long)mm * a.ldo + n] = v;
+                            if (a.gran)
+                                __hip_atomic_store(a.gran + n, ((unsigned long long)gtag << 32) | (unsigned long long)__float_as_uint(v),
+                                                   __ATOMIC_RELAXED, __HIP_MEMORY_SCOPE_AGENT);
+                        }
+                    }
+                }
+            }
+        }
+    }
+}
+
+}
diff --git a/umgen_amd/csrc/kernels.h b/umgen_amd/csrc/kernels.h
--- a/umgen_amd/csrc/kernels.h
+++ b/umgen_amd/csrc/kernels.h
@@ -67,6 +67,7 @@
     void* cache; long scene_stride; const int* d_len; int Lmax;
     int rows_per_block;
     int E;
+    unsigned long long* gran; const unsigned* d_tag;
 };
 template <typename T> void launch_gemv(hipStream_t s, const GemvArgs& a);
 
```

Result: no change. 1973 scene-tokens/s, median of 4 (+0.0%).
